# SakodaShintaro/f2-nerf

Measured on AMD Instinct MI355X. Metric: rendered rays/sec (fwd+bwd) at 800x800, higher is better.
Workload: dtype f32; 1 GPU; ngp_fox-like synthetic views 800x800, 128 samples/ray, L=16 F=2 T=2^19, 65536-ray chunks, TRAIN render + loss + backward (optimizer excluded); pixel_order=rows, regime=dense

## Files before the change

### f2-nerf_amd/csrc/host/ragged_ops.cpp

```cpp
#include "ragged_ops.hpp"

#include "kernel_timer.hpp"

using torch::Tensor;
using torch::autograd::AutogradContext;
using torch::autograd::variable_list;

namespace
{

class FlexSumFn : public torch::autograd::Function<FlexSumFn>
{
public:
  static variable_list forward(AutogradContext * ctx, Tensor val, Tensor idx)
  {
    val = f2n::dev_f32(val, "FlexOps::Sum val");
    idx = f2n::dev_i32(idx, "FlexOps::Sum idx_start_end");
    TORCH_CHECK(val.dim() == 1 || val.dim() == 2, "FlexOps::Sum expects [n] or [n, c]");
    const int n_rays = (int)idx.size(0);
    void * s = f2n::current_stream(val);
    Tensor sum;
    if (val.dim() == 1) {
      sum = torch::empty({n_rays}, val.options());
      f2n::check(
        f2n_seg_sum_fwd(f2n::fptr(val), f2n::iptr(idx), sum.data_ptr<float>(), n_rays, s),
        "f2n_seg_sum_fwd");
    } else {
      const int vec = (int)val.size(1);
      sum = torch::empty({n_rays, vec}, val.options());
      f2n::check(
        f2n_seg_sum_vec_fwd(f2n::fptr(val), f2n::iptr(idx), sum.data_ptr<float>(), n_rays, vec, s),
        "f2n_seg_sum_vec_fwd");
    }
    ctx->save_for_backward({idx});
    ctx->saved_data["n_all"] = (int64_t)val.size(0);
    ctx->saved_data["vec"] = (int64_t)(val.dim() == 1 ? 0 : val.size(1));
    return {sum};
  }

  static variable_list backward(AutogradContext * ctx, variable_list grad_output)
  {
    Tensor dsum = f2n::dev_f32(grad_output[0], "FlexOps::Sum grad");
    Tensor idx = ctx->get_saved_variables()[0];
    const int64_t n_all = ctx->saved_data["n_all"].toInt();
    const int vec = (int)ctx->saved_data["vec"].toInt();
    const int n_rays = (int)idx.size(0);
    void * s = f2n::current_stream(dsum);
    Tensor dval;
    if (vec == 0) {
      dval = torch::zeros({n_all}, dsum.options());
      f2n::check(
        f2n_seg_sum_bwd(f2n::fptr(dsum), f2n::iptr(idx), dval.data_ptr<float>(), n_rays, s),
        "f2n_seg_sum_bwd");
    } else {
      dval = torch::zeros({n_all, vec}, dsum.options());
      f2n::check(
        f2n_seg_sum_vec_bwd(f2n::fptr(dsum), f2n::iptr(idx), dval.data_ptr<float>(), n_rays, vec, s),
        "f2n_seg_sum_vec_bwd");
    }
    return {dval, Tensor()};
  }
};

class FlexAccumulateSumFn : public torch::autograd::Function<FlexAccumulateSumFn>
{
public:
  static variable_list forward(AutogradContext * ctx, Tensor val, Tensor idx, bool include_this)
  {
    val = f2n::dev_f32(val, "FlexOps::AccumulateSum val");
    idx = f2n::dev_i32(idx, "FlexOps::AccumulateSum idx_start_end");
    TORCH_CHECK(val.dim() == 1, "FlexOps::AccumulateSum expects [n]");
    Tensor sum = torch::zeros_like(val);
    f2n::check(
      f2n_seg_scan_fwd(
        f2n::fptr(val), f2n::iptr(idx), sum.data_ptr<float>(), (int)idx.size(0), include_this,
        f2n::current_stream(val)),
      "f2n_seg_scan_fwd");
    ctx->save_for_backward({idx});
    ctx->saved_data["include_this"] = include_this;
    return {sum};
  }

  static variable_list backward(AutogradContext * ctx, variable_list grad_output)
  {
    Tensor dsum = f2n::dev_f32(grad_output[0], "FlexOps::AccumulateSum grad");
    Tensor idx = ctx->get_saved_variables()[0];
    const bool include_this = ctx->saved_data["include_this"].toBool();
    Tensor dval = torch::zeros_like(dsum);
    f2n::check(
      f2n_seg_scan_bwd(
        f2n::fptr(dsum), f2n::iptr(idx), dval.data_ptr<float>(), (int)idx.size(0), include_this,
        f2n::current_stream(dsum)),
      "f2n_seg_scan_bwd");
    return {dval, Tensor(), Tensor()};
  }
};

class WeightVarFn : public torch::autograd::Function<WeightVarFn>
{
public:
  static variable_list forward(AutogradContext * ctx, Tensor weights, Tensor idx)
  {
    weights = f2n::dev_f32(weights, "CustomOps::WeightVar weights");
    idx = f2n::dev_i32(idx, "CustomOps::WeightVar idx_start_end");
    const int n_rays = (int)idx.size(0);
    Tensor out = torch::empty({n_rays}, weights.options());
    f2n::check(
      f2n_weight_var_fwd(
        f2n::fptr(weights), f2n::iptr(idx), out.data_ptr<float>(), n_rays,
        f2n::current_stream(weights)),
      "f2n_weight_var_fwd");
    ctx->save_for_backward({weights, idx});
    return {out};
  }

  static variable_list backward(AutogradContext * ctx, variable_list grad_output)
  {
    Tensor dvar = f2n::dev_f32(grad_output[0], "CustomOps::WeightVar grad");
    auto saved = ctx->get_saved_variables();
    Tensor & weights = saved[0];
    Tensor & idx = saved[1];
    Tensor dw = torch::zeros_like(weights);
    f2n::check(
      f2n_weight_var_bwd(
        f2n::fptr(weights), f2n::iptr(idx), f2n::fptr(dvar), dw.data_ptr<float>(),
        (int)idx.size(0), f2n::current_stream(dvar)),
      "f2n_weight_var_bwd");
    return {dw, Tensor()};
  }
};

class ScatterAddFn : public torch::autograd::Function<ScatterAddFn>
{
public:
  static variable_list forward(AutogradContext * ctx, Tensor emb, Tensor idx, Tensor to_add)
  {
    emb = f2n::dev_f32(emb, "CustomOps::ScatterAdd emb");
    idx = f2n::dev_i32(idx, "CustomOps::ScatterAdd idx");
    to_add = f2n::dev_f32(to_add, "CustomOps::ScatterAdd to_add");
    const int64_t n_all = idx.size(0);
    const int C = (int)emb.size(1);
    TORCH_CHECK(to_add.size(0) == n_all && to_add.size(1) == C, "ScatterAdd shape mismatch");
    Tensor sum = torch::empty_like(to_add);
    f2n::check(
      f2n_scatter_add_fwd(
        f2n::fptr(emb), f2n::iptr(idx), f2n::fptr(to_add), sum.data_ptr<float>(), n_all, C,
        f2n::current_stream(to_add)),
      "f2n_scatter_add_fwd");
    ctx->save_for_backward({idx});
    ctx->saved_data["n_emb"] = (int64_t)emb.size(0);
    return {sum};
  }

  static variable_list backward(AutogradContext * ctx, variable_list grad_output)
  {
    Tensor dsum = f2n::dev_f32(grad_output[0], "CustomOps::ScatterAdd grad");
    Tensor idx = ctx->get_saved_variables()[0];
    const int n_emb = (int)ctx->saved_data["n_emb"].toInt();
    const int C = (int)dsum.size(1);
    Tensor demb = torch::empty({n_emb, C}, dsum.options());
    f2n::check(
      f2n_scatter_add_bwd(
        f2n::iptr(idx), f2n::fptr(dsum), demb.data_ptr<float>(), idx.size(0), n_emb, C,
        f2n::current_stream(dsum)),
      "f2n_scatter_add_bwd");
    return {demb, Tensor(), dsum};
  }
};

class CompositeFn : public torch::autograd::Function<CompositeFn>
{
public:
  static variable_list forward(
    AutogradContext * ctx, Tensor field_out, Tensor rgb, Tensor dt, Tensor t, Tensor idx, Tensor bg,
    bool tiled)
  {
    field_out = f2n::dev_f32(field_out, "composite field_out");
    rgb = f2n::dev_f32(rgb, "composite rgb");
    dt = f2n::dev_f32(dt, "composite dt");
    t = f2n::dev_f32(t, "composite t");
    idx = f2n::dev_i32(idx, "composite idx_start_end");
    bg = f2n::dev_f32(bg, "composite bg_color");
    TORCH_CHECK(field_out.dim() == 2 && rgb.dim() == 2 && rgb.size(1) == 3, "composite shapes");
    const int64_t n = field_out.size(0);
    const int n_rays = (int)idx.size(0);
    auto opt = field_out.options();
    Tensor colors = torch::empty({n_rays, 3}, opt), depths = torch::empty({n_rays}, opt);
    Tensor weights = tiled ? torch::empty({n}, opt) : torch::zeros({n}, opt);
    Tensor last_trans = torch::empty({n_rays}, opt);
    ctx->saved_data["tiled"] = tiled;
    f2n::check(
      f2n_composite_fwd(
        f2n::fptr(field_out), field_out.size(1), f2n::fptr(rgb), f2n::fptr(dt), f2n::fptr(t),
        f2n::iptr(idx), f2n::fptr(bg), colors.data_ptr<float>(), depths.data_ptr<float>(),
        weights.data_ptr<float>(), last_trans.data_ptr<float>(), n_rays, 3.f, 1e-2f,
        f2n::current_stream(field_out)),
      "f2n_composite_fwd");
    ctx->save_for_backward({field_out, rgb, dt, t, idx, bg, weights, last_trans});
    return {colors, depths, weights};
  }

  static variable_list backward(AutogradContext * ctx, variable_list grad_output)
  {
    auto sv = ctx->get_saved_variables();
    Tensor &field_out = sv[0], &rgb = sv[1], &dt = sv[2], &t = sv[3], &idx = sv[4], &bg = sv[5],
           &weights = sv[6], &last_trans = sv[7];
    const int n_rays = (int)idx.size(0);
    const int64_t n = field_out.size(0);
    auto opt = field_out.options();
    Tensor d_colors = grad_output[0].defined() ? f2n::dev_f32(grad_output[0], "d_colors")
                                               : torch::zeros({n_rays, 3}, opt);
    Tensor d_depths = grad_output[1].defined() ? f2n::dev_f32(grad_output[1], "d_depths")
                                               : torch::zeros({n_rays}, opt);
    Tensor d_weights =
      grad_output[2].defined() ? f2n::dev_f32(grad_output[2], "d_weights") : Tensor();
    const bool tiled = ctx->saved_data["tiled"].toBool();
    Tensor d_logit = tiled ? torch::empty({n}, opt) : torch::zeros({n}, opt);
    Tensor d_rgb = tiled ? torch::empty({n, 3}, opt) : torch::zeros({n, 3}, opt);
    f2n::check(
      f2n_composite_bwd(
        f2n::fptr(field_out), field_out.size(1), f2n::fptr(rgb), f2n::fptr(dt), f2n::fptr(t),
        f2n::iptr(idx), f2n::fptr(bg), f2n::fptr(weights), f2n::fptr(last_trans),
        f2n::fptr(d_colors), f2n::fptr(d_depths), f2n::fptr(d_weights), d_logit.data_ptr<float>(),
        d_rgb.data_ptr<float>(), n_rays, 3.f, 1e-2f, f2n::current_stream(field_out)),
      "f2n_composite_bwd");
    if (field_out.size(1) == 1)
      return {d_logit.unsqueeze(1), d_rgb, Tensor(), Tensor(), Tensor(), Tensor(), Tensor()};
    Tensor d_field = torch::zeros_like(field_out);
    d_field.select(1, 0).copy_(d_logit);
    return {d_field, d_rgb, Tensor(), Tensor(), Tensor(), Tensor(), Tensor()};
  }
};

Tensor as_channel_major(const Tensor & t)
{
  if (t.dim() == 2 && t.stride(0) == 1 && t.stride(1) == t.size(0)) return t.t();
  return t.t().contiguous();
}

class ShadeFn : public torch::autograd::Function<ShadeFn>
{
public:
  static variable_list forward(
    AutogradContext * ctx, Tensor enc, Tensor dirs, Tensor sample_img, Tensor w_h, Tensor b_h,
    Tensor w1, Tensor b1, Tensor w2, Tensor b2, Tensor app_emb)
  {
    TORCH_CHECK(enc.is_cuda() && enc.scalar_type() == torch::kFloat32 && enc.dim() == 2, "enc");
    const int64_t n = enc.size(0);
    const int C = (int)enc.size(1);
    Tensor enc_cm = as_channel_major(enc);
    dirs = f2n::dev_f32(dirs.detach(), "shade dirs");
    const bool use_emb = sample_img.defined() && app_emb.defined() && sample_img.numel() > 0 &&
                         app_emb.numel() > 0;
    if (use_emb) sample_img = f2n::dev_i32(sample_img, "shade sample_img");
    w_h = f2n::dev_f32(w_h, "w_h");
    b_h = f2n::dev_f32(b_h, "b_h");
    w1 = f2n::dev_f32(w1, "w1");
    b1 = f2n::dev_f32(b1, "b1");
    w2 = f2n::dev_f32(w2, "w2");
    b2 = f2n::dev_f32(b2, "b2");
    Tensor emb = use_emb ? f2n::dev_f32(app_emb, "app_emb") : Tensor();
    TORCH_CHECK(
      w_h.size(0) == 16 && w_h.size(1) == C && w1.size(0) == 64 && w1.size(1) == 32 &&
        w2.size(0) == 3 && w2.size(1) == 64,
      "shade: layer shapes must be 16xC, 64x32, 3x64");
    Tensor logit = torch::empty({n}, enc.options()), rgb = torch::empty({n, 3}, enc.options());
    {
    f2n::ScopedKernelTimer timer("shade_fwd", f2n::current_stream(enc_cm), (double)n);
    f2n::check(
      f2n_shade_fwd(
        enc_cm.data_ptr<float>(), C, dirs.data_ptr<float>(), use_emb ? f2n::iptr(sample_img) : nullptr,
        f2n::fptr(w_h), f2n::fptr(b_h), f2n::fptr(w1), f2n::fptr(b1), f2n::fptr(w2), f2n::fptr(b2),
        f2n::fptr(emb), logit.data_ptr<float>(), rgb.data_ptr<float>(),
        nullptr,
        n, f2n::current_stream(enc_cm)),
      "f2n_shade_fwd");
    }
    ctx->save_for_backward(
      {enc_cm, dirs, use_emb ? sample_img : Tensor(), w_h, b_h, w1, b1, w2, b2, emb});
    return {logit, rgb};
  }

  static variable_list backward(AutogradContext * ctx, variable_list grad_output)
  {
    auto sv = ctx->get_saved_variables();
    Tensor &enc_cm = sv[0], &dirs = sv[1], &sample_img = sv[2], &w_h = sv[3], &b_h = sv[4],
           &w1 = sv[5], &b1 = sv[6], &w2 = sv[7], &b2 = sv[8], &emb = sv[9];
    const int C = (int)enc_cm.size(0);
    const int64_t n = enc_cm.size(1);
    auto opt = enc_cm.options();
    Tensor d_logit = grad_output[0].defined() ? f2n::dev_f32(grad_output[0], "d_logit")
                                              : torch::zeros({n}, opt);
    Tensor d_rgb = grad_output[1].defined() ? f2n::dev_f32(grad_output[1], "d_rgb")
                                            : torch::zeros({n, 3}, opt);
    Tensor d_enc_cm = torch::empty({(int64_t)C, n}, opt);
    const bool use_emb = emb.defined() && sample_img.defined();
    auto pad4 = [](int64_t v) { return (v + 3) / 4 * 4; };
    const int64_t sizes[7] = {w_h.numel(), b_h.numel(), w1.numel(), b1.numel(),
                              w2.numel(), b2.numel(), use_emb ? emb.numel() : 0};
    int64_t total = 0;
    for (int64_t v : sizes) total += pad4(v);
    Tensor gbuf = torch::zeros({total}, opt);
    int64_t off = 0;
    auto take = [&](const Tensor & like, int64_t numel) {
      Tensor v = gbuf.narrow(0, off, numel).view(like.sizes());
      off += pad4(numel);
      return v;
    };
    Tensor g_w_h = take(w_h, sizes[0]), g_b_h = take(b_h, sizes[1]), g_w1 = take(w1, sizes[2]),
           g_b1 = take(b1, sizes[3]), g_w2 = take(w2, sizes[4]), g_b2 = take(b2, sizes[5]);
    Tensor g_emb = use_emb ? take(emb, sizes[6]) : Tensor();
    {
    f2n::ScopedKernelTimer timer("shade_bwd", f2n::current_stream(enc_cm), (double)n);
    f2n::check(
      f2n_shade_bwd(
        enc_cm.data_ptr<float>(), C, dirs.data_ptr<float>(), use_emb ? f2n::iptr(sample_img) : nullptr,
        f2n::fptr(w_h), f2n::fptr(b_h), f2n::fptr(w1), f2n::fptr(b1), f2n::fptr(w2), f2n::fptr(b2),
        f2n::fptr(emb), f2n::fptr(d_logit), f2n::fptr(d_rgb), d_enc_cm.data_ptr<float>(),
        g_w_h.data_ptr<float>(), g_b_h.data_ptr<float>(), g_w1.data_ptr<float>(),
        g_b1.data_ptr<float>(), g_w2.data_ptr<float>(), g_b2.data_ptr<float>(),
        use_emb ? g_emb.data_ptr<float>() : nullptr, nullptr, n,
        f2n::current_stream(enc_cm)),
      "f2n_shade_bwd");
    }
    return {d_enc_cm.t(), Tensor(), Tensor(), g_w_h, g_b_h, g_w1, g_b1, g_w2, g_b2, g_emb};
  }
};


class TrainLossFn : public torch::autograd::Function<TrainLossFn>
{
public:
  static variable_list forward(
    AutogradContext * ctx, Tensor colors, Tensor gt, Tensor var, double var_weight)
  {
    colors = f2n::dev_f32(colors, "train_loss colors");
    gt = f2n::dev_f32(gt, "train_loss gt_colors");
    var = f2n::dev_f32(var, "train_loss var");
    const int64_t n_rays = colors.size(0);
    TORCH_CHECK(
      colors.dim() == 2 && colors.size(1) == 3 && gt.sizes() == colors.sizes() &&
        var.numel() == n_rays && n_rays > 0 && n_rays <= INT32_MAX,
      "train_loss: colors/gt [n_rays,3], var [n_rays]");
    Tensor d_colors = torch::empty_like(colors), d_var = torch::empty({n_rays}, colors.options());
    Tensor partial = torch::empty({f2n_loss_workspace_floats((int)n_rays)}, colors.options());
    Tensor out = torch::empty({4}, colors.options());
    f2n::check(
      f2n_loss_fwd(
        colors.data_ptr<float>(), gt.data_ptr<float>(), var.data_ptr<float>(), (int)n_rays,
        (float)var_weight, d_colors.data_ptr<float>(), d_var.data_ptr<float>(),
        partial.data_ptr<float>(), out.data_ptr<float>(), f2n::current_stream(colors)),
      "f2n_loss_fwd");
    ctx->save_for_backward({d_colors, d_var});
    ctx->saved_data["var_shape"] = var.sizes().vec();
    return {out};
  }

  static variable_list backward(AutogradContext * ctx, variable_list grad_output)
  {
    auto sv = ctx->get_saved_variables();
    Tensor g = grad_output[0].select(0, 0);
    Tensor d_var = (sv[1] * g).view(ctx->saved_data["var_shape"].toIntVector());
    return {sv[0] * g, Tensor(), d_var, Tensor()};
  }
};

}

namespace torch::autograd
{

variable_list TruncExp::forward(AutogradContext * ctx, Tensor input)
{
  ctx->save_for_backward({input});
  return {torch::exp(input)};
}

variable_list TruncExp::backward(AutogradContext * ctx, variable_list grad_output)
{
  Tensor x = ctx->get_saved_variables()[0];
  return {grad_output[0] * torch::exp(x.clamp(-100.f, 5.f))};
}

}

Tensor FlexOps::Sum(Tensor val, Tensor idx_start_end)
{
  return FlexSumFn::apply(val.contiguous(), idx_start_end.contiguous())[0];
}

Tensor FlexOps::AccumulateSum(Tensor val, Tensor idx_start_end, bool include_this)
{
  return FlexAccumulateSumFn::apply(val.contiguous(), idx_start_end.contiguous(), include_this)[0];
}

Tensor CustomOps::WeightVar(Tensor weights, Tensor idx_start_end)
{
  return WeightVarFn::apply(weights.contiguous(), idx_start_end.contiguous())[0];
}

Tensor CustomOps::ScatterAdd(Tensor emb, Tensor idx, Tensor to_add)
{
  return ScatterAddFn::apply(emb, idx, to_add)[0];
}

Tensor CustomOps::ScatterIdx(int n_all_pts, Tensor idx_start_end, Tensor emb_idx)
{
  idx_start_end = f2n::dev_i32(idx_start_end, "CustomOps::ScatterIdx idx_start_end");
  emb_idx = f2n::dev_i32(emb_idx, "CustomOps::ScatterIdx emb_idx");
  Tensor ret = torch::empty({n_all_pts}, idx_start_end.options());
  f2n::check(
    f2n_scatter_idx(
      f2n::iptr(idx_start_end), f2n::iptr(emb_idx), ret.data_ptr<int32_t>(),
      (int)idx_start_end.size(0), f2n::current_stream(idx_start_end)),
    "f2n_scatter_idx");
  return ret;
}

f2n::ShadeOut f2n::shade(
  const Tensor & enc, const Tensor & dirs, const Tensor & sample_img, const Tensor & w_h,
  const Tensor & b_h, const Tensor & w1, const Tensor & b1, const Tensor & w2, const Tensor & b2,
  const Tensor & app_emb)
{
  const Tensor no_img = torch::empty({0}, f2n::int_on(enc.device()));
  const Tensor no_emb = torch::empty({0, 16}, enc.options());
  const bool use_emb = sample_img.defined() && app_emb.defined();
  auto out = ShadeFn::apply(
    enc, dirs, use_emb ? sample_img : no_img, w_h, b_h, w1, b1, w2, b2, use_emb ? app_emb : no_emb);
  return {out[0], out[1]};
}

f2n::CompositeOut f2n::composite(
  const Tensor & field_out, const Tensor & rgb, const Tensor & dt, const Tensor & t,
  const Tensor & idx_start_end, const Tensor & bg_color, bool bounds_tile_samples)
{
  auto out = CompositeFn::apply(field_out, rgb, dt, t, idx_start_end, bg_color, bounds_tile_samples);
  return {out[0], out[1], out[2]};
}

Tensor f2n::train_loss(
  const Tensor & colors, const Tensor & gt_colors, const Tensor & var, float var_loss_weight)
{
  return TrainLossFn::apply(colors, gt_colors, var, (double)var_loss_weight)[0];
}
```

### f2-nerf_amd/csrc/host/ragged_ops.hpp

```cpp
#pragma once

#include "common.hpp"

namespace torch::autograd
{

class TruncExp : public Function<TruncExp>
{
public:
  static variable_list forward(AutogradContext * ctx, Tensor input);
  static variable_list backward(AutogradContext * ctx, variable_list grad_output);
};

}

namespace FlexOps
{
torch::Tensor Sum(torch::Tensor val, torch::Tensor idx_start_end);
torch::Tensor AccumulateSum(torch::Tensor val, torch::Tensor idx_start_end, bool include_this);
}

namespace CustomOps
{
torch::Tensor WeightVar(torch::Tensor weights, torch::Tensor idx_start_end);
torch::Tensor ScatterAdd(torch::Tensor emb, torch::Tensor idx, torch::Tensor to_add);
torch::Tensor ScatterIdx(int n_all_pts, torch::Tensor idx_start_end, torch::Tensor emb_idx);
}

namespace f2n
{

struct CompositeOut
{
  Tensor colors;
  Tensor depths;
  Tensor weights;
};

CompositeOut composite(
  const Tensor & field_out, const Tensor & rgb, const Tensor & dt, const Tensor & t,
  const Tensor & idx_start_end, const Tensor & bg_color, bool bounds_tile_samples = false);


struct ShadeOut
{
  Tensor logit;
  Tensor rgb;
};

ShadeOut shade(
  const Tensor & enc, const Tensor & dirs, const Tensor & sample_img, const Tensor & w_h,
  const Tensor & b_h, const Tensor & w1, const Tensor & b1, const Tensor & w2, const Tensor & b2,
  const Tensor & app_emb);

Tensor train_loss(
  const Tensor & colors, const Tensor & gt_colors, const Tensor & var, float var_loss_weight);

inline bool shade_supported(int64_t C) { return C == 8 || C == 16 || C == 32 || C == 64; }

}
```

### f2-nerf_amd/csrc/host/renderer.cpp

```cpp
#include "renderer.hpp"

#include "kernel_timer.hpp"

#include "ragged_ops.hpp"
#include "rays.hpp"

#include <c10/hip/HIPGuard.h>
#include <hip/hip_runtime_api.h>

using Tensor = torch::Tensor;

f2n::HostCount::~HostCount()
{
  if (event_) hipEventDestroy((hipEvent_t)event_);
  if (pinned_) hipHostFree(pinned_);
}

void f2n::HostCount::request(const torch::Tensor & device_int32, void * stream)
{
  TORCH_CHECK(
    device_int32.is_cuda() && device_int32.scalar_type() == torch::kInt32 && device_int32.numel() == 1,
    "HostCount: one int32 on the device");
  const int device = (int)device_int32.device().index();
  c10::hip::HIPGuard on_device(device);
  if (pending_) {
    hipEventSynchronize((hipEvent_t)event_);
    pending_ = false;
  }
  if (!pinned_)
    TORCH_CHECK(hipHostMalloc((void **)&pinned_, sizeof(int32_t), hipHostMallocDefault) == hipSuccess,
                "HostCount: pinned allocation failed");
  if (!event_ || device_ != device) {
    if (event_) hipEventDestroy((hipEvent_t)event_);
    hipEvent_t ev;
    TORCH_CHECK(hipEventCreateWithFlags(&ev, hipEventDisableTiming) == hipSuccess,
                "HostCount: event creation failed");
    event_ = ev;
    device_ = device;
  }
  TORCH_CHECK(
    hipMemcpyAsync(pinned_, device_int32.data_ptr<int32_t>(), sizeof(int32_t), hipMemcpyDeviceToHost,
                   (hipStream_t)stream) == hipSuccess &&
      hipEventRecord((hipEvent_t)event_, (hipStream_t)stream) == hipSuccess,
    "HostCount: copy failed");
  pending_ = true;
}

int64_t f2n::HostCount::wait()
{
  TORCH_CHECK(pending_, "HostCount: wait() without request()");
  TORCH_CHECK(hipEventSynchronize((hipEvent_t)event_) == hipSuccess, "HostCount: wait failed");
  pending_ = false;
  return (int64_t)*pinned_;
}


namespace
{

std::pair<Tensor, Tensor> bounds_from_counts(const Tensor & counts, void * stream)
{
  const int n = (int)counts.size(0);
  Tensor bounds = torch::empty({n, 2}, counts.options()), total = torch::empty({1}, counts.options());
  f2n::check(
    f2n_bounds_from_counts(
      counts.data_ptr<int32_t>(), bounds.data_ptr<int32_t>(), total.data_ptr<int32_t>(), n, stream),
    "f2n_bounds_from_counts");
  return {bounds, total};
}

class RayUnpermuteFn : public torch::autograd::Function<RayUnpermuteFn>
{
public:
  static torch::autograd::variable_list forward(
    torch::autograd::AutogradContext * ctx, Tensor colors, Tensor depths, Tensor weights,
    Tensor perm, Tensor inv, Tensor bounds_sorted, Tensor bounds_caller, int64_t S, bool rows)
  {
    colors = f2n::dev_f32(colors, "colors");
    depths = f2n::dev_f32(depths, "depths");
    weights = f2n::dev_f32(weights, "weights");
    const int n = (int)perm.size(0);
    void * s = f2n::current_stream(colors);
    Tensor c = torch::empty_like(colors), d = torch::empty_like(depths), w = torch::empty_like(weights);
    gather(colors, depths, weights, c, d, w, inv, bounds_sorted, bounds_caller, n, S, rows, s);
    ctx->save_for_backward({perm, bounds_sorted, bounds_caller});
    ctx->saved_data["S"] = S;
    ctx->saved_data["rows"] = rows;
    return {c, d, w};
  }

  static torch::autograd::variable_list backward(
    torch::autograd::AutogradContext * ctx, torch::autograd::variable_list g)
  {
    auto saved = ctx->get_saved_variables();
    const Tensor & perm = saved[0];
    const int n = (int)perm.size(0);
    const int64_t S = ctx->saved_data["S"].toInt();
    const bool rows = ctx->saved_data["rows"].toBool();
    Tensor gc = g[0].defined() ? f2n::dev_f32(g[0], "grad colors") : Tensor();
    Tensor gd = g[1].defined() ? f2n::dev_f32(g[1], "grad depths") : Tensor();
    Tensor gw = g[2].defined() ? f2n::dev_f32(g[2], "grad weights") : Tensor();
    Tensor dc = gc.defined() ? torch::empty_like(gc) : Tensor();
    Tensor dd = gd.defined() ? torch::empty_like(gd) : Tensor();
    Tensor dw = gw.defined() ? torch::empty_like(gw) : Tensor();
    void * s = f2n::current_stream(perm);
    gather(gc, gd, gw, dc, dd, dw, perm, saved[2], saved[1], n, S, rows, s);
    return {dc, dd, dw, Tensor(), Tensor(), Tensor(), Tensor(), Tensor(), Tensor()};
  }

private:
  static void gather(
    const Tensor & c, const Tensor & d, const Tensor & w, Tensor & c_out, Tensor & d_out,
    Tensor & w_out, const Tensor & map, const Tensor & src_b, const Tensor & dst_b, int n, int64_t S,
    bool rows, void * s)
  {
    const int32_t * m = map.data_ptr<int32_t>();
    if (c.defined())
      f2n::check(f2n_gather_rows(f2n::fptr(c), c_out.data_ptr<float>(), m, n, 3, s), "f2n_gather_rows");
    if (d.defined())
      f2n::check(f2n_gather_rows(f2n::fptr(d), d_out.data_ptr<float>(), m, n, 1, s), "f2n_gather_rows");
    if (!w.defined()) return;
    if (rows)
      f2n::check(
        f2n_gather_rows(f2n::fptr(w), w_out.data_ptr<float>(), m, n, (int)S, s), "f2n_gather_rows");
    else
      f2n::check(
        f2n_gather_segments(
          f2n::fptr(w), f2n::iptr(src_b), w_out.data_ptr<float>(), f2n::iptr(dst_b), m, n, s),
        "f2n_gather_segments");
  }
};

class RayGradFn : public torch::autograd::Function<RayGradFn>
{
public:
  static torch::autograd::variable_list forward(
    torch::autograd::AutogradContext * ctx, Tensor enc, Tensor rays_o, Tensor rays_d, Tensor pts,
    Tensor t, Tensor bounds, torch::IValue hash3d_info)
  {
    Hash3DAnchored * field = hash3d_info.toCustomClass<Hash3DAnchoredInfo>()->hash3d_;
    ctx->saved_data["hash3d_info"] = hash3d_info;
    ctx->saved_data["n_rays"] = rays_o.size(0);
    ctx->save_for_backward(
      {f2n::dev_f32(pts.detach(), "kept pts"), f2n::dev_f32(t.detach(), "kept t"),
       f2n::dev_i32(bounds, "kept bounds"), f2n::dev_f32(rays_d.detach(), "rays_d"),
       field->table_f16()});
    return {enc};
  }

  static torch::autograd::variable_list backward(
    torch::autograd::AutogradContext * ctx, torch::autograd::variable_list grad)
  {
    const Tensor & g_enc = grad[0];
    const bool want_o = ctx->needs_input_grad(1), want_d = ctx->needs_input_grad(2);
    Tensor d_o, d_d;
    if (want_o || want_d) {
      auto sv = ctx->get_saved_variables();
      const Tensor &pts = sv[0], &t = sv[1], &bounds = sv[2], &rays_d = sv[3], &table16 = sv[4];
      const int64_t n_rays = ctx->saved_data["n_rays"].toInt();
      d_o = torch::empty({n_rays, 3}, rays_d.options());
      d_d = torch::empty({n_rays, 3}, rays_d.options());
      if (!g_enc.defined()) {
        d_o.zero_();
        d_d.zero_();
      } else {
        Hash3DAnchored * field =
          ctx->saved_data["hash3d_info"].toCustomClass<Hash3DAnchoredInfo>()->hash3d_;
        const int64_t n = pts.size(0);
        const int L = (int)field->options_.n_levels, F = (int)field->options_.n_channels;
        const auto [g, ld_point, ld_chan] = f2n::encoding_grad_strides(g_enc, n, (int64_t)L * F);
        void * stream = f2n::current_stream(pts);
        f2n::ScopedKernelTimer timer("hash_rays_grad", stream, (double)n);
        f2n::check(
          f2n_hash_rays_grad(
            pts.data_ptr<float>(), t.data_ptr<float>(), bounds.data_ptr<int32_t>(),
            rays_d.data_ptr<float>(), reinterpret_cast<const uint16_t *>(table16.data_ptr()),
            field->prim_pool_.data_ptr<int32_t>(), field->bias_pool_.data_ptr<float>(),
            field->level_mul_.data_ptr<float>(), g.data_ptr<float>(), ld_point, ld_chan,
            d_o.data_ptr<float>(), d_d.data_ptr<float>(), (int)n_rays, L, F,
            (uint32_t)field->local_size_, field->level_stride_, 128.f ,
            stream),
          "f2n_hash_rays_grad");
      }
    }
    return {g_enc, want_o ? d_o : Tensor(), want_d ? d_d : Tensor(), Tensor(), Tensor(), Tensor(),
            Tensor()};
  }
};

}

Tensor f2n::ray_order(const Tensor & rays_d_in)
{
  const Tensor rays_d = f2n::dev_f32(rays_d_in.detach(), "rays_d");
  TORCH_CHECK(rays_d.dim() == 2 && rays_d.size(1) == 3, "rays_d must be [n, 3]");
  const int n = (int)rays_d.size(0);
  Tensor keys = torch::empty({n}, f2n::int_on(rays_d.device()));
  f2n::check(
    f2n_ray_keys(rays_d.data_ptr<float>(), keys.data_ptr<int32_t>(), n, f2n::current_stream(rays_d)),
    "f2n_ray_keys");
  return std::get<1>(keys.sort(true, 0, false));
}

Renderer::Renderer(int n_images, const RendererOptions & opt) : options_(opt)
{
  pts_sampler_ = std::make_shared<PtsSampler>(opt.sampler);

  scene_field_ = std::make_shared<Hash3DAnchored>(opt.field);
  register_module("scene_field", scene_field_);

  shader_ = std::make_shared<SHShader>(opt.field.device);
  register_module("shader", shader_);

  app_emb_ = torch::randn({n_images, 16}, f2n::float_on(opt.field.device)) * .1f;
  app_emb_.requires_grad_(true);
  register_parameter("app_emb", app_emb_);
}

RenderResult Renderer::render(
  const Tensor & rays_o, const Tensor & rays_d, const Tensor & emb_idx, RunningMode mode)
{
  return render(rays_o, rays_d, emb_idx, mode, Tensor(), Tensor());
}

RenderResult Renderer::render(
  const Tensor & rays_o, const Tensor & rays_d, const Tensor & emb_idx, RunningMode mode,
  const Tensor & noise_in, const Tensor & bg_in)
{
  const int64_t n_rays = rays_o.size(0);
  const auto fopt = f2n::float_on(rays_o.device());
  Tensor noise = noise_in.defined() ? noise_in
                                    : pts_sampler_->draw_noise(n_rays, mode, rays_o.device());
  Tensor bg_color = bg_in.defined() ? bg_in
                    : (mode == RunningMode::TRAIN) ? torch::rand({n_rays, 3}, fopt)
                                                   : torch::ones({n_rays, 3}, fopt) * .5f;
  if (n_rays <= 0) {
    record_kept(0);
    return {bg_color, torch::zeros({n_rays}, fopt), torch::full({n_rays}, 512.f, fopt), Tensor()};
  }
  const Route route = choose_route(rays_o, rays_d, bg_color);
  RenderResult res = route.first_pass == Route::OpByOp
                       ? render_op_by_op(rays_o, rays_d, emb_idx, mode, noise, bg_color, route)
                       : render_fused(rays_o, rays_d, emb_idx, mode, noise, bg_color, route);
  if (options_.check_finite) CHECK(std::isfinite(res.colors.mean().item<float>()));
  return res;
}

Renderer::Route Renderer::choose_route(
  const Tensor & rays_o, const Tensor & rays_d, const Tensor & bg_color) const
{
  Route route;
  const auto & field = scene_field_->options_;
  route.fused_net = options_.fused_shade && f2n::shade_supported(field.n_levels * field.n_channels) &&
                    field.mlp_out_dim == 16;
  const bool rays_need_grad =
    torch::GradMode::is_enabled() && (rays_o.requires_grad() || rays_d.requires_grad());
  if (rays_need_grad) route.grad_rays = Rays{rays_o, rays_d};
  if (!options_.fused || (rays_need_grad && !(options_.fused_ray_grad && route.fused_net)))
    route.first_pass = Route::OpByOp;
  else if (occupancy_)
    route.first_pass = Route::March;
  else if (route.fused_net && (options_.dense_first_pass == 1 ||
                               (options_.dense_first_pass < 0 && last_kept_fraction_ > 0.4f)))
    route.first_pass = Route::Dense;
  else
    route.first_pass = Route::March;
  route.bucketed = route.first_pass == Route::Dense &&
                   rays_o.size(0) >= options_.ray_order_min_rays &&
                   f2n_get_option(F2N_OPT_RAY_ORDER) == 0 && !rays_need_grad &&
                   !(torch::GradMode::is_enabled() && bg_color.requires_grad());
  return route;
}

void Renderer::record_kept(int64_t n_kept, int64_t n_all)
{
  last_n_samples_ = n_kept;
  if (n_all >= 0) last_kept_fraction_ = n_all > 0 ? (float)n_kept / (float)n_all : 0.f;
}


RenderResult Renderer::render_op_by_op(
  const Tensor & rays_o, const Tensor & rays_d, const Tensor & emb_idx, RunningMode mode,
  const Tensor & noise, const Tensor & bg_color, const Route & route)
{
  const int64_t n_rays = rays_o.size(0);
  const int64_t S = pts_sampler_->options_.max_samples;
  SampleResultFlex all = route.grad_rays.origins.defined()
                           ? pts_sampler_->get_samples_aten(rays_o, rays_d, noise)
                           : pts_sampler_->get_samples(rays_o, rays_d, noise);

  auto density_act = [](const Tensor & x) {
    return torch::autograd::TruncExp::apply(x - 3.f)[0];
  };

  SampleResultFlex kept;
  {
    Tensor scene_feat = scene_field_->query(all.pts);
    Tensor density = density_act(scene_feat.index({Slc(), Slc(0, 1)}));
    Tensor sec = density.index({Slc(), 0}) * all.dt;
    Tensor occupied;
    if (occupancy_) {
      occupied = occupancy_->occupied(all.pts);
      sec = sec * occupied.to(sec.scalar_type());
    }
    Tensor acc = FlexOps::AccumulateSum(sec, all.pts_idx_bounds, false);
    Tensor mask = torch::exp(-acc) > options_.early_stop_trans;
    if (occupancy_) mask = mask.logical_and(occupied);
    Tensor mask_idx = torch::where(mask)[0];
    kept.pts = all.pts.index({mask_idx}).contiguous();
    kept.dirs = all.dirs.index({mask_idx}).contiguous();
    kept.dt = all.dt.index({mask_idx}).contiguous();
    kept.t = all.t.index({mask_idx}).contiguous();
    Tensor num = mask.reshape({n_rays, S}).sum(1);
    Tensor cum = torch::cumsum(num, 0);
    kept.pts_idx_bounds = torch::stack({cum - num, cum}, 1).to(torch::kInt32).contiguous();
  }
  record_kept(kept.pts.size(0));

  Tensor scene_feat = scene_field_->query(kept.pts);
  Tensor density = density_act(scene_feat.index({Slc(), Slc(0, 1)}));
  Tensor sampled_colors = shade_aten(scene_feat, kept, emb_idx, mode);
  Tensor sampled_t = (kept.t + 1e-2f).contiguous();
  Tensor sec = density.index({Slc(), 0}) * kept.dt;
  Tensor alphas = 1.f - torch::exp(-sec);
  Tensor idx = kept.pts_idx_bounds;
  Tensor trans = torch::exp(-FlexOps::AccumulateSum(sec, idx, false));
  Tensor weights = trans * alphas;
  Tensor last_trans = torch::exp(-FlexOps::Sum(sec, idx));
  Tensor colors = FlexOps::Sum(weights.unsqueeze(-1) * sampled_colors, idx) +
                  last_trans.unsqueeze(-1) * bg_color;
  Tensor depths = FlexOps::Sum(weights * sampled_t, idx) / (1.f - last_trans + 1e-4f);
  return {colors, depths, weights, idx};
}


RenderResult Renderer::render_fused(
  const Tensor & rays_o_raw, const Tensor & rays_d_raw, const Tensor & emb_idx, RunningMode mode,
  const Tensor & noise_raw, const Tensor & bg_color, const Route & route)
{
  Tensor rays_o = f2n::dev_f32(rays_o_raw.detach(), "rays_o");
  Tensor rays_d = f2n::dev_f32(rays_d_raw.detach(), "rays_d");
  Tensor noise = noise_raw.defined() ? f2n::dev_f32(noise_raw, "noise") : Tensor();
  const int n_rays = (int)rays_o.size(0);
  const int S = pts_sampler_->options_.max_samples;
  TORCH_CHECK(!noise.defined() || noise.numel() == (int64_t)n_rays * S, "noise shape");
  if (route.first_pass == Route::Dense)
    return route.bucketed
             ? render_dense_bucketed(rays_o, rays_d, emb_idx, mode, noise, bg_color, route)
             : render_dense(rays_o, rays_d, emb_idx, mode, noise, bg_color, route);

  void * stream = f2n::current_stream(rays_o);
  Hash3DAnchored & field = *scene_field_;
  SampleResultFlex kept;
  {
    torch::NoGradGuard no_grad;
    Tensor table16 = field.table_f16();
    auto head = field.density_head();
    Tensor counts = torch::empty({n_rays}, f2n::int_on(rays_o.device()));
    Tensor len;
    if (occupancy_) {
      TORCH_CHECK(
        occupancy_->words().device() == rays_o.device(), "the occupancy grid lives on another device");
      len = torch::empty_like(counts);
      f2n::ScopedKernelTimer timer("density_march_occ", stream, (double)n_rays);
      f2n::check(
        f2n_density_march_occ(
          rays_o.data_ptr<float>(), rays_d.data_ptr<float>(), f2n::fptr(noise),
          reinterpret_cast<const uint16_t *>(table16.data_ptr()),
          field.prim_pool_.data_ptr<int32_t>(), field.bias_pool_.data_ptr<float>(),
          field.level_mul_.data_ptr<float>(), head.first.data_ptr<float>(),
          head.second.data_ptr<float>(), occupancy_->words_ptr(), (int)occupancy_->resolution(),
          counts.data_ptr<int32_t>(), len.data_ptr<int32_t>(), n_rays, S,
          pts_sampler_->options_.step, (int)field.options_.n_levels, (int)field.options_.n_channels,
          (uint32_t)field.local_size_, field.level_stride_, options_.early_stop_trans, 3.f, stream),
        "f2n_density_march_occ");
    } else {
      f2n::ScopedKernelTimer timer("density_march", stream, (double)n_rays);
      f2n::check(
      f2n_density_march(
        rays_o.data_ptr<float>(), rays_d.data_ptr<float>(), f2n::fptr(noise),
        reinterpret_cast<const uint16_t *>(table16.data_ptr()), field.prim_pool_.data_ptr<int32_t>(),
        field.bias_pool_.data_ptr<float>(), field.level_mul_.data_ptr<float>(),
        head.first.data_ptr<float>(), head.second.data_ptr<float>(), counts.data_ptr<int32_t>(),
        n_rays, S, pts_sampler_->options_.step, (int)field.options_.n_levels,
        (int)field.options_.n_channels, (uint32_t)field.local_size_, field.level_stride_,
        options_.early_stop_trans, 3.f, stream),
      "f2n_density_march");
    }
    auto [bounds, total] = bounds_from_counts(counts, stream);
    const int64_t n_kept = total.item<int>();
    record_kept(n_kept, (int64_t)n_rays * S);
    kept = compact_samples(rays_o, rays_d, noise, bounds, n_kept, len);
  }
  return shade_and_composite(kept, emb_idx, mode, bg_color, route);
}

RenderResult Renderer::render_dense_bucketed(
  const Tensor & rays_o, const Tensor & rays_d, const Tensor & emb_idx_in, RunningMode mode,
  const Tensor & noise, const Tensor & bg_in, const Route & route)
{
  const int n_rays = (int)rays_o.size(0);
  const int64_t S = pts_sampler_->options_.max_samples;
  const auto iopt = f2n::int_on(rays_o.device());
  void * stream = f2n::current_stream(rays_o);
  const Tensor emb_idx = (mode == RunningMode::TRAIN && emb_idx_in.defined())
                           ? f2n::dev_i32(emb_idx_in, "emb_idx") : Tensor();
  const Tensor bg = f2n::dev_f32(bg_in.detach(), "bg_color");
  TORCH_CHECK(bg.numel() == (int64_t)n_rays * 3, "bg_color shape");
  TORCH_CHECK(!emb_idx.defined() || emb_idx.numel() == n_rays, "emb_idx shape");

  const Tensor order = f2n::ray_order(rays_d);
  Tensor perm = torch::empty({n_rays}, iopt), inv = torch::empty({n_rays}, iopt);
  Tensor o_p = torch::empty_like(rays_o), d_p = torch::empty_like(rays_d), bg_p = torch::empty_like(bg);
  Tensor emb_p = emb_idx.defined() ? torch::empty_like(emb_idx) : Tensor();
  Tensor noise_p = noise.defined() ? torch::empty_like(noise) : Tensor();
  f2n::check(
    f2n_ray_permute(
      order.data_ptr<int64_t>(), n_rays, (int)S, rays_o.data_ptr<float>(), rays_d.data_ptr<float>(),
      f2n::iptr(emb_idx), bg.data_ptr<float>(), f2n::fptr(noise), perm.data_ptr<int32_t>(),
      o_p.data_ptr<float>(), d_p.data_ptr<float>(),
      emb_idx.defined() ? emb_p.data_ptr<int32_t>() : nullptr, bg_p.data_ptr<float>(),
      f2n::fptr_mut(noise_p), inv.data_ptr<int32_t>(), stream),
    "f2n_ray_permute");
  RenderResult r = render_dense(o_p, d_p, emb_p, mode, noise_p, bg_p, route);

  const bool rows = r.weights.size(0) == (int64_t)n_rays * S;
  Tensor bounds = r.idx_start_end;
  if (!rows) {
    Tensor counts = torch::empty({n_rays}, iopt);
    f2n::check(
      f2n_counts_through(
        r.idx_start_end.data_ptr<int32_t>(), inv.data_ptr<int32_t>(), counts.data_ptr<int32_t>(),
        n_rays, stream),
      "f2n_counts_through");
    bounds = bounds_from_counts(counts, stream).first;
  }
  auto out = RayUnpermuteFn::apply(
    r.colors, r.depths, r.weights, perm, inv, r.idx_start_end, bounds, S, rows);
  return {out[0], out[1], out[2], bounds};
}

RenderResult Renderer::render_dense(
  const Tensor & rays_o, const Tensor & rays_d, const Tensor & emb_idx, RunningMode mode,
  const Tensor & noise, const Tensor & bg_color, const Route & route)
{
  const int n_rays = (int)rays_o.size(0);
  const int S = pts_sampler_->options_.max_samples;
  void * stream = f2n::current_stream(rays_o);
  Hash3DAnchored & field = *scene_field_;
  SampleResultFlex all = pts_sampler_->get_samples(rays_o, rays_d, noise);
  const int64_t n_all = all.pts.size(0);
  Tensor contracted_all, enc_all_cm;
  {
    torch::NoGradGuard no_grad;
    enc_all_cm = field.encode(all.pts, S, &contracted_all).t();
    TORCH_CHECK(enc_all_cm.is_contiguous(), "encode() must return channel-major storage");
  }

  if (options_.deferred_check) {
    Tensor total = scan_survivors(all, enc_all_cm, n_rays).second;
    if (!deferred_bad_.defined()) deferred_bad_ = torch::zeros({1}, total.options());
    deferred_bad_.add_(total.ne(n_all).to(torch::kInt32));
    record_kept(n_all, n_all);
    return shade_and_composite(all, emb_idx, mode, bg_color, route, enc_all_cm, contracted_all);
  }

  const bool may_guess = options_.speculate_dense && last_kept_fraction_ >= 1.f && n_all > 0;
  const bool large = n_all >= options_.margin_min_samples;
  if (may_guess && large) {
    if (auto guess = shade_all_unless_near_threshold(
          all, emb_idx, mode, bg_color, route, enc_all_cm, contracted_all)) {
      record_kept(n_all, n_all);
      return *guess;
    }
  }

  auto [bounds, total] = scan_survivors(all, enc_all_cm, n_rays);
  survivors_.request(total, stream);
  RenderResult guess;
  const bool guessed = may_guess && !large;
  if (guessed)
    guess = shade_and_composite(all, emb_idx, mode, bg_color, route, enc_all_cm, contracted_all);
  const int64_t n_kept = survivors_.wait();
  record_kept(n_kept, n_all);
  if (guessed && n_kept == n_all) return guess;
  guess = RenderResult();
  if (n_kept == n_all) {
    all.pts_idx_bounds = bounds;
    return shade_and_composite(all, emb_idx, mode, bg_color, route, enc_all_cm, contracted_all);
  }
  SampleResultFlex kept = compact_samples(rays_o, rays_d, noise, bounds, n_kept);
  const int64_t C = enc_all_cm.size(0);
  Tensor enc_kept_cm = torch::empty({C, n_kept}, rays_o.options());
  f2n::check(
    f2n_compact_rows_cm(
      enc_all_cm.data_ptr<float>(), n_all, enc_kept_cm.data_ptr<float>(), n_kept, (int)C,
      bounds.data_ptr<int32_t>(), n_rays, S, stream),
    "f2n_compact_rows_cm");
  return shade_and_composite(kept, emb_idx, mode, bg_color, route, enc_kept_cm);
}

bool Renderer::deferred_check_ok()
{
  if (!deferred_bad_.defined()) return true;
  const bool ok = deferred_bad_.item<int32_t>() == 0;
  deferred_bad_.zero_();
  return ok;
}


std::pair<Tensor, Tensor> Renderer::scan_survivors(
  const SampleResultFlex & all, const Tensor & enc_all_cm, int n_rays)
{
  torch::NoGradGuard no_grad;
  void * stream = f2n::current_stream(enc_all_cm);
  auto head = scene_field_->density_head();
  Tensor counts = torch::empty({n_rays}, f2n::int_on(enc_all_cm.device()));
  {
    f2n::ScopedKernelTimer timer("density_scan", stream, (double)n_rays);
    f2n::check(
      f2n_density_scan(
        enc_all_cm.data_ptr<float>(), (int)enc_all_cm.size(0), all.dt.data_ptr<float>(),
        head.first.data_ptr<float>(), head.second.data_ptr<float>(), counts.data_ptr<int32_t>(),
        n_rays, pts_sampler_->options_.max_samples, options_.early_stop_trans, 3.f, stream),
      "f2n_density_scan");
  }
  return bounds_from_counts(counts, stream);
}

SampleResultFlex Renderer::compact_samples(
  const Tensor & rays_o, const Tensor & rays_d, const Tensor & noise, const Tensor & bounds,
  int64_t n_kept, const Tensor & len)
{
  const auto fopt = rays_o.options();
  SampleResultFlex kept{
    torch::empty({n_kept, 3}, fopt), torch::empty({n_kept, 3}, fopt), torch::empty({n_kept}, fopt),
    torch::empty({n_kept}, fopt), bounds};
  if (len.defined()) {
    f2n::check(
      f2n_sample_compact_occ(
        rays_o.data_ptr<float>(), rays_d.data_ptr<float>(), f2n::fptr(noise),
        bounds.data_ptr<int32_t>(), len.data_ptr<int32_t>(), occupancy_->words_ptr(),
        (int)occupancy_->resolution(), kept.pts.data_ptr<float>(), kept.dirs.data_ptr<float>(),
        kept.dt.data_ptr<float>(), kept.t.data_ptr<float>(), (int)rays_o.size(0),
        pts_sampler_->options_.max_samples, pts_sampler_->options_.step,
        f2n::current_stream(rays_o)),
      "f2n_sample_compact_occ");
    return kept;
  }
  f2n::check(
    f2n_sample_compact(
      rays_o.data_ptr<float>(), rays_d.data_ptr<float>(), f2n::fptr(noise),
      bounds.data_ptr<int32_t>(), kept.pts.data_ptr<float>(), kept.dirs.data_ptr<float>(),
      kept.dt.data_ptr<float>(), kept.t.data_ptr<float>(), (int)rays_o.size(0),
      pts_sampler_->options_.max_samples, pts_sampler_->options_.step,
      f2n::current_stream(rays_o)),
    "f2n_sample_compact");
  return kept;
}

std::optional<RenderResult> Renderer::shade_all_unless_near_threshold(
  const SampleResultFlex & all, const Tensor & emb_idx, RunningMode mode, const Tensor & bg_color,
  const Route & route, const Tensor & enc_cm, const Tensor & contracted)
{
  void * stream = f2n::current_stream(all.pts);
  Tensor near_threshold = torch::zeros({1}, f2n::int_on(all.pts.device()));
  Shaded shaded = shade(all, emb_idx, mode, route, enc_cm, contracted);
  const int S = pts_sampler_->options_.max_samples;
  const float limit = -std::log(options_.early_stop_trans) - 0.5f;
  f2n::check(
    f2n_density_margin(
      shaded.field_out.data_ptr<float>(), all.dt.data_ptr<float>(),
      near_threshold.data_ptr<int32_t>(), (int)(all.pts.size(0) / S), S, 3.f, limit, stream),
    "f2n_density_margin");
  survivors_.request(near_threshold, stream);
  RenderResult guess = composite(all, shaded, bg_color, route);
  if (survivors_.wait() != 0) return std::nullopt;
  return guess;
}

RenderResult Renderer::shade_and_composite(
  const SampleResultFlex & kept, const Tensor & emb_idx, RunningMode mode, const Tensor & bg_color,
  const Route & route, const Tensor & enc_cm, const Tensor & contracted)
{
  return composite(kept, shade(kept, emb_idx, mode, route, enc_cm, contracted), bg_color, route);
}

Renderer::Shaded Renderer::shade(
  const SampleResultFlex & kept, const Tensor & emb_idx, RunningMode mode, const Route & route,
  const Tensor & enc_cm, const Tensor & contracted)
{
  if (!route.fused_net) {
    Tensor scene_feat = scene_field_->query(kept.pts);
    return {scene_feat, shade_aten(scene_feat, kept, emb_idx, mode)};
  }
  const int64_t n_kept = kept.pts.size(0);
  Tensor enc = enc_cm.defined() ? scene_field_->encode_cached(kept.pts, enc_cm, contracted)
                                : scene_field_->encode(kept.pts);
  if (route.grad_rays.origins.defined()) {
    auto info = torch::make_intrusive<Hash3DAnchoredInfo>();
    info->hash3d_ = scene_field_.get();
    enc = RayGradFn::apply(
      enc, route.grad_rays.origins, route.grad_rays.dirs, kept.pts, kept.t, kept.pts_idx_bounds,
      torch::IValue(info))[0];
  }
  Tensor sample_img;
  if (mode == RunningMode::TRAIN)
    sample_img = CustomOps::ScatterIdx((int)n_kept, kept.pts_idx_bounds, emb_idx);
  auto mlp = shader_->mlp_params();
  f2n::ShadeOut sh = f2n::shade(
    enc, kept.dirs, sample_img, scene_field_->mlp_->weight, scene_field_->mlp_->bias, mlp[0],
    mlp[1], mlp[2], mlp[3], mode == RunningMode::TRAIN ? app_emb_ : Tensor());
  return {sh.logit.unsqueeze(1), sh.rgb};
}

Tensor Renderer::shade_aten(
  const Tensor & scene_feat, const SampleResultFlex & kept, const Tensor & emb_idx, RunningMode mode)
{
  const int64_t n_kept = kept.pts.size(0);
  Tensor shading_feat = torch::cat(
    {torch::ones({n_kept, 1}, scene_feat.options()),
     scene_feat.index({Slc(), Slc(1, torch::indexing::None)})},
    1);
  if (mode == RunningMode::TRAIN) {
    Tensor all_emb_idx = CustomOps::ScatterIdx((int)n_kept, kept.pts_idx_bounds, emb_idx);
    shading_feat = CustomOps::ScatterAdd(app_emb_, all_emb_idx, shading_feat);
  }
  return shader_->query(shading_feat, kept.dirs);
}

RenderResult Renderer::composite(
  const SampleResultFlex & kept, const Shaded & shaded, const Tensor & bg_color, const Route & route)
{
  f2n::CompositeOut out = f2n::composite(
    shaded.field_out, shaded.rgb, kept.dt, kept.t, kept.pts_idx_bounds, bg_color, route.fused_net);
  return {out.colors, out.depths, out.weights, kept.pts_idx_bounds};
}


std::tuple<Tensor, Tensor> Renderer::render_all_rays(
  const Tensor & rays_o, const Tensor & rays_d, const int batch_size)
{
  const int64_t n_rays = rays_d.size(0);
  std::vector<Tensor> colors, depths;
  for (int64_t lo = 0; lo < n_rays; lo += batch_size) {
    const int64_t hi = std::min<int64_t>(lo + batch_size, n_rays);
    RenderResult r = render(
      rays_o.index({Slc(lo, hi)}).contiguous(), rays_d.index({Slc(lo, hi)}).contiguous(), Tensor(),
      RunningMode::VALIDATE);
    colors.push_back(r.colors);
    depths.push_back(r.depths.reshape({-1, 1}));
  }
  return {torch::cat(colors, 0), torch::cat(depths, 0)};
}

std::tuple<Tensor, Tensor> Renderer::render_image(
  const Tensor & pose, const Tensor & intrinsic, const int h, const int w, const int batch_size)
{
  Rays rays = get_view_rays(pose, intrinsic, h, w);
  const int B = options_.pixel_tiles;
  Tensor order;
  if (B > 1 && h % B == 0 && w % B == 0) {
    order = torch::arange((int64_t)h * w, torch::TensorOptions().dtype(torch::kInt64).device(pose.device()))
              .view({h / B, B, w / B, B})
              .permute({0, 2, 1, 3})
              .reshape({-1});
    rays.origins = rays.origins.index_select(0, order);
    rays.dirs = rays.dirs.index_select(0, order);
  }
  auto [colors, depths] = render_all_rays(rays.origins, rays.dirs, batch_size);
  if (order.defined()) {
    colors = torch::empty_like(colors).index_copy_(0, order, colors);
    depths = torch::empty_like(depths).index_copy_(0, order, depths);
  }
  colors = colors.reshape({h, w, 3}).clip(0.f, 1.f);
  depths = depths.reshape({h, w, 1}).repeat({1, 1, 3});
  return {colors, depths};
}

std::vector<torch::optim::OptimizerParamGroup> Renderer::optim_param_groups(float lr)
{
  std::vector<torch::optim::OptimizerParamGroup> groups;
  for (auto & g : scene_field_->optim_param_groups(lr)) groups.emplace_back(g);
  for (auto & g : shader_->optim_param_groups(lr)) groups.emplace_back(g);
  auto opt = std::make_unique<torch::optim::AdamOptions>(lr);
  opt->betas(std::make_tuple(0.9, 0.99)).eps(1e-15).weight_decay(1e-6);
  groups.emplace_back(std::vector<Tensor>{app_emb_}, std::move(opt));
  return groups;
}


f2n::TrainStepResult f2n::train_step(
  Renderer & renderer, const Tensor & rays_o, const Tensor & rays_d, const Tensor & emb_idx,
  const Tensor & gt_colors, float var_loss_weight, const Tensor & noise, const Tensor & bg_color,
  bool run_backward)
{
  RenderResult res =
    renderer.render(rays_o, rays_d, emb_idx, RunningMode::TRAIN, noise, bg_color);
  Tensor var = CustomOps::WeightVar(res.weights, res.idx_start_end);
  if (var_loss_weight == 0.f) var = var.detach();
  Tensor stats = f2n::train_loss(res.colors, gt_colors, var, var_loss_weight);
  Tensor loss = stats[0];
  TrainStepResult out;
  out.loss = loss.detach();
  out.sq_err_sum = stats[3].detach();
  out.n_values = res.colors.numel();
  out.n_samples = renderer.last_n_samples_;
  if (run_backward && loss.requires_grad()) loss.backward();
  return out;
}
```

### f2-nerf_amd/csrc/kernels/shade.hip

```cpp
#include "sh_basis.hiph"
#include "shade_mfma.hiph"

#include <cstdlib>
#include <cstring>

namespace
{

constexpr int kOut1 = 16;
constexpr int kIn2 = 32;
constexpr int kHid = 64;
constexpr float kEps = 1e-3f;

struct ShadeParams
{
  const float * __restrict__ w_h;
  const float * __restrict__ b_h;
  const float * __restrict__ w1;
  const float * __restrict__ b1;
  const float * __restrict__ w2;
  const float * __restrict__ b2;
  const float * __restrict__ emb;
};

template <int C>
__device__ __forceinline__ void shade_forward(
  const float (&e)[C], float dx, float dy, float dz, const float * __restrict__ emb_row,
  const ShadeParams & P, float (&h)[kOut1], float (&X)[kIn2], float (&pre)[kHid], float (&o)[3])
{
#pragma unroll
  for (int i = 0; i < kOut1; i++) {
    float acc = P.b_h[i];
#pragma unroll
    for (int c = 0; c < C; c++) acc = fmaf(e[c], P.w_h[i * C + c], acc);
    h[i] = acc;
  }
  X[0] = 1.f;
#pragma unroll
  for (int i = 1; i < kOut1; i++) X[i] = h[i];
  if (emb_row) {
#pragma unroll
    for (int i = 0; i < kOut1; i++) X[i] += emb_row[i];
  }
  sh_basis<4>(dx, dy, dz, &X[kOut1]);
#pragma unroll
  for (int j = 0; j < kHid; j++) {
    float acc = P.b1[j];
#pragma unroll
    for (int i = 0; i < kIn2; i++) acc = fmaf(X[i], P.w1[j * kIn2 + i], acc);
    pre[j] = acc;
  }
#pragma unroll
  for (int c = 0; c < 3; c++) {
    float acc = P.b2[c];
#pragma unroll
    for (int j = 0; j < kHid; j++) acc = fmaf(fmaxf(pre[j], 0.f), P.w2[c * kHid + j], acc);
    o[c] = acc;
  }
}

template <int C>
__global__ __launch_bounds__(F2N_BLOCK) void shade_fwd_kernel(
  const float * __restrict__ enc, const float * __restrict__ dirs,
  const int32_t * __restrict__ sample_img, const float * __restrict__ p_w_h,
  const float * __restrict__ p_b_h, const float * __restrict__ p_w1,
  const float * __restrict__ p_b1, const float * __restrict__ p_w2,
  const float * __restrict__ p_b2, const float * __restrict__ p_emb, float * __restrict__ logit,
  float * __restrict__ rgb, float * __restrict__ pre_out, int64_t n)
{
  const int64_t p = (int64_t)blockIdx.x * F2N_BLOCK + threadIdx.x;
  if (p >= n) return;
  const ShadeParams P{p_w_h, p_b_h, p_w1, p_b1, p_w2, p_b2, p_emb};
  float e[C];
#pragma unroll
  for (int c = 0; c < C; c++) e[c] = enc[(int64_t)c * n + p];
  const float * emb_row = (P.emb && sample_img) ? P.emb + (int64_t)sample_img[p] * kOut1 : nullptr;
  float h[kOut1], X[kIn2], pre[kHid], o[3];
  shade_forward<C>(e, dirs[3 * p], dirs[3 * p + 1], dirs[3 * p + 2], emb_row, P, h, X, pre, o);
  logit[p] = h[0];
#pragma unroll
  for (int c = 0; c < 3; c++)
    rgb[3 * p + c] = (1.f + 2.f * kEps) / (1.f + expf(-o[c])) - kEps;
  if (pre_out) {
#pragma unroll
    for (int j = 0; j < kHid; j++) pre_out[(int64_t)j * n + p] = pre[j];
  }
}


constexpr int kTP = 65;
constexpr int kDoOff = kHid * kTP;
constexpr int kHP = kOut1 + 4;

template <int C>
struct BwdShape
{
  static constexpr int kERowP = C + 4;
  static constexpr int kHOff = 64 * kERowP;
  static constexpr int kTile =
    (kHOff + 64 * kHP > kDoOff + 64 * 3) ? kHOff + 64 * kHP : kDoOff + 64 * 3;
  static constexpr int kWeights = kOut1 * (C + 4) + kHid * (kIn2 + 4) + kHid * 4 + 4;
  static constexpr int kWaves = ((kWeights + 8 * kTile) * 4 <= 160 * 1024) ? 8 : 4;
};

__device__ __forceinline__ void wave_lds_sync()
{
  __builtin_amdgcn_fence(__ATOMIC_RELEASE, "wavefront");
  __builtin_amdgcn_wave_barrier();
  __builtin_amdgcn_fence(__ATOMIC_ACQUIRE, "wavefront");
}

template <int C>
__global__ __launch_bounds__(BwdShape<C>::kWaves * 64) void shade_bwd_kernel(
  const float * __restrict__ enc, const float * __restrict__ dirs,
  const int32_t * __restrict__ sample_img, const float * __restrict__ p_w_h,
  const float * __restrict__ p_b_h, const float * __restrict__ p_w1,
  const float * __restrict__ p_b1, const float * __restrict__ p_w2,
  const float * __restrict__ p_b2, const float * __restrict__ p_emb,
  const float * __restrict__ d_logit, const float * __restrict__ d_rgb, float * __restrict__ d_enc,
  float * __restrict__ g_w_h, float * __restrict__ g_b_h, float * __restrict__ g_w1,
  float * __restrict__ g_b1, float * __restrict__ g_w2, float * __restrict__ g_b2,
  float * __restrict__ g_emb, const float * __restrict__ pre_in, int64_t n)
{
  static_assert(C % 4 == 0 && C <= kHid, "C must be a multiple of 4 and at most 64");
  constexpr int kBwdWaves = BwdShape<C>::kWaves;
  constexpr int kWavelds = BwdShape<C>::kTile;
  constexpr int kWhP = C + 4, kW1P = kIn2 + 4;
  constexpr int kOffWh = 0, kOffW1 = kOffWh + kOut1 * kWhP, kOffW2T = kOffW1 + kHid * kW1P,
                kOffB2 = kOffW2T + kHid * 4, kWTotal = kOffB2 + 4;
  __shared__ __attribute__((aligned(16))) float lds_all[kWTotal + kBwdWaves * kWavelds];
  float * lds_w = lds_all;
  float * lds = lds_all + kWTotal;
  for (int i = threadIdx.x; i < kOut1 * C; i += kBwdWaves * 64)
    lds_w[kOffWh + (i / C) * kWhP + (i % C)] = p_w_h[i];
  for (int i = threadIdx.x; i < kHid * kIn2; i += kBwdWaves * 64)
    lds_w[kOffW1 + (i / kIn2) * kW1P + (i % kIn2)] = p_w1[i];
  for (int i = threadIdx.x; i < 3 * kHid; i += kBwdWaves * 64)
    lds_w[kOffW2T + (i % kHid) * 4 + (i / kHid)] = p_w2[i];
  if (threadIdx.x < kOut1) lds_w[kOffWh + threadIdx.x * kWhP + C] = p_b_h[threadIdx.x];
  if (threadIdx.x < kHid) {
    lds_w[kOffW1 + threadIdx.x * kW1P + kIn2] = p_b1[threadIdx.x];
    lds_w[kOffW2T + threadIdx.x * 4 + 3] = 0.f;
  }
  if (threadIdx.x < 4) lds_w[kOffB2 + threadIdx.x] = (threadIdx.x < 3) ? p_b2[threadIdx.x] : 0.f;
  __syncthreads();

  const int lane = lane_id();
  const int wave = (int)(threadIdx.x >> 6);
  int vzero;
  asm volatile("v_mov_b32 %0, 0" : "=v"(vzero));
  float * tileP = lds + wave * kWavelds;
  const bool has_emb = (p_emb != nullptr) && (sample_img != nullptr);

  float acc_w1[kIn2];
  float acc_b1 = 0.f;
  float acc_w2[3];
  constexpr int CQ = C / 4;
  float acc_wh[CQ];
  float acc_bh[kOut1];
  float acc_b2[3];
#pragma unroll
  for (int i = 0; i < kIn2; i++) acc_w1[i] = 0.f;
#pragma unroll
  for (int c = 0; c < 3; c++) acc_w2[c] = acc_b2[c] = 0.f;
#pragma unroll
  for (int k = 0; k < CQ; k++) acc_wh[k] = 0.f;
#pragma unroll
  for (int i = 0; i < kOut1; i++) acc_bh[i] = 0.f;

  const int64_t n_strides = (n + 63) / 64;
  const int64_t wave_global = (int64_t)blockIdx.x * kBwdWaves + wave;
  const int64_t wave_count = (int64_t)gridDim.x * kBwdWaves;
  for (int64_t st = wave_global; st < n_strides; st += wave_count) {
    const int64_t p = st * 64 + lane;
    const bool valid = p < n;
    const int64_t pc = valid ? p : n - 1;

    float e[C];
#pragma unroll
    for (int c = 0; c < C; c++) e[c] = enc[(int64_t)c * n + pc];
    const int img = has_emb ? sample_img[pc] : 0;
    float X[kIn2];
    {
#pragma unroll 2
      for (int i = 0; i < kOut1; i++) {
        const float * row = lds_w + kOffWh + (i + vzero) * kWhP;
        float acc = row[C];
#pragma unroll
        for (int c = 0; c < C; c += 4) {
          const float4 w = *reinterpret_cast<const float4 *>(row + c);
          acc = fmaf(e[c], w.x, acc);
          acc = fmaf(e[c + 1], w.y, acc);
          acc = fmaf(e[c + 2], w.z, acc);
          acc = fmaf(e[c + 3], w.w, acc);
        }
        tileP[i * 64 + lane] = acc;
      }
      X[0] = 1.f;
#pragma unroll
      for (int i = 1; i < kOut1; i++) X[i] = tileP[i * 64 + lane];
      if (has_emb) {
        const float * emb_row = p_emb + (int64_t)img * kOut1;
#pragma unroll
        for (int i = 0; i < kOut1; i++) X[i] += emb_row[i];
      }
      sh_basis<4>(dirs[3 * pc], dirs[3 * pc + 1], dirs[3 * pc + 2], &X[kOut1]);
    }
    float o[3];
    {
      const float4 b2 = *reinterpret_cast<const float4 *>(lds_w + kOffB2);
      o[0] = b2.x;
      o[1] = b2.y;
      o[2] = b2.z;
      if (pre_in) {
#pragma unroll 8
        for (int j = 0; j < kHid; j++) {
          const float acc = pre_in[(int64_t)j * n + pc];
          tileP[j * kTP + lane] = acc;
          const float hj = fmaxf(acc, 0.f);
          const float4 w2 = *reinterpret_cast<const float4 *>(lds_w + kOffW2T + (j + vzero) * 4);
          o[0] = fmaf(hj, w2.x, o[0]);
          o[1] = fmaf(hj, w2.y, o[1]);
          o[2] = fmaf(hj, w2.z, o[2]);
        }
      } else {
#pragma unroll 2
        for (int j = 0; j < kHid; j++) {
          const float * row = lds_w + kOffW1 + (j + vzero) * kW1P;
          float acc = row[kIn2];
#pragma unroll
          for (int i = 0; i < kIn2; i += 4) {
            const float4 w = *reinterpret_cast<const float4 *>(row + i);
            acc = fmaf(X[i], w.x, acc);
            acc = fmaf(X[i + 1], w.y, acc);
            acc = fmaf(X[i + 2], w.z, acc);
            acc = fmaf(X[i + 3], w.w, acc);
          }
          tileP[j * kTP + lane] = acc;
          const float hj = fmaxf(acc, 0.f);
          const float4 w2 = *reinterpret_cast<const float4 *>(lds_w + kOffW2T + (j + vzero) * 4);
          o[0] = fmaf(hj, w2.x, o[0]);
          o[1] = fmaf(hj, w2.y, o[1]);
          o[2] = fmaf(hj, w2.z, o[2]);
        }
      }
    }

    float d_o[3];
#pragma unroll
    for (int c = 0; c < 3; c++) {
      const float sg = 1.f / (1.f + expf(-o[c]));
      const float g = valid ? d_rgb[3 * pc + c] : 0.f;
      d_o[c] = g * (1.f + 2.f * kEps) * sg * (1.f - sg);
      acc_b2[c] += d_o[c];
    }

    tileP[kDoOff + lane * 3 + 0] = d_o[0];
    tileP[kDoOff + lane * 3 + 1] = d_o[1];
    tileP[kDoOff + lane * 3 + 2] = d_o[2];
    wave_lds_sync();
#pragma unroll 4
    for (int s = 0; s < 64; s++) {
      const float a = fmaxf(tileP[lane * kTP + s], 0.f);
      const float * g = tileP + kDoOff + (s + vzero) * 3;
      acc_w2[0] = fmaf(g[0], a, acc_w2[0]);
      acc_w2[1] = fmaf(g[1], a, acc_w2[1]);
      acc_w2[2] = fmaf(g[2], a, acc_w2[2]);
    }
    wave_lds_sync();

    float dX[kOut1];
#pragma unroll
    for (int i = 0; i < kOut1; i++) dX[i] = 0.f;
#pragma unroll 2
    for (int j = 0; j < kHid; j++) {
      const float pre = tileP[j * kTP + lane];
      const float4 w2 = *reinterpret_cast<const float4 *>(lds_w + kOffW2T + (j + vzero) * 4);
      float dh = d_o[0] * w2.x;
      dh = fmaf(d_o[1], w2.y, dh);
      dh = fmaf(d_o[2], w2.z, dh);
      dh = (pre > 0.f) ? dh : 0.f;
      tileP[j * kTP + lane] = dh;
      const float * row = lds_w + kOffW1 + (j + vzero) * kW1P;
#pragma unroll
      for (int i = 0; i < kOut1; i += 4) {
        const float4 w = *reinterpret_cast<const float4 *>(row + i);
        dX[i] = fmaf(dh, w.x, dX[i]);
        dX[i + 1] = fmaf(dh, w.y, dX[i + 1]);
        dX[i + 2] = fmaf(dh, w.z, dX[i + 2]);
        dX[i + 3] = fmaf(dh, w.w, dX[i + 3]);
      }
    }
    float d_h[kOut1];
    d_h[0] = valid ? d_logit[pc] : 0.f;
#pragma unroll
    for (int i = 1; i < kOut1; i++) d_h[i] = dX[i];
#pragma unroll
    for (int i = 0; i < kOut1; i++) acc_bh[i] += d_h[i];

    wave_lds_sync();
#pragma unroll 2
    for (int s = 0; s < 64; s++) {
      const float a = tileP[lane * kTP + s];
      acc_b1 += a;
#pragma unroll
      for (int i = 0; i < kIn2; i++) {
        const float xs =
          __int_as_float(__builtin_amdgcn_readlane(__float_as_int(X[i]), s));
        acc_w1[i] = fmaf(a, xs, acc_w1[i]);
      }
    }
    wave_lds_sync();

    {
      float d_e[C];
#pragma unroll
      for (int c = 0; c < C; c++) d_e[c] = 0.f;
#pragma unroll
      for (int i = 0; i < kOut1; i++) tileP[i * 64 + lane] = d_h[i];
#pragma unroll 2
      for (int i = 0; i < kOut1; i++) {
        const float a = tileP[i * 64 + lane];
        const float * row = lds_w + kOffWh + (i + vzero) * kWhP;
#pragma unroll
        for (int c = 0; c < C; c += 4) {
          const float4 w = *reinterpret_cast<const float4 *>(row + c);
          d_e[c] = fmaf(a, w.x, d_e[c]);
          d_e[c + 1] = fmaf(a, w.y, d_e[c + 1]);
          d_e[c + 2] = fmaf(a, w.z, d_e[c + 2]);
          d_e[c + 3] = fmaf(a, w.w, d_e[c + 3]);
        }
      }
      if (valid) {
#pragma unroll
        for (int c = 0; c < C; c++) d_enc[(int64_t)c * n + p] = d_e[c];
      }
    }

    {
      constexpr int kEP = BwdShape<C>::kERowP;
      float * rowsH = tileP + BwdShape<C>::kHOff;
      wave_lds_sync();
#pragma unroll
      for (int c = 0; c < C; c += 4)
        *reinterpret_cast<float4 *>(tileP + lane * kEP + c) =
          make_float4(e[c], e[c + 1], e[c + 2], e[c + 3]);
      *reinterpret_cast<float4 *>(rowsH + lane * kHP) =
        make_float4(valid ? dX[0] : 0.f, d_h[1], d_h[2], d_h[3]);
#pragma unroll
      for (int i = 4; i < kOut1; i += 4)
        *reinterpret_cast<float4 *>(rowsH + lane * kHP + i) =
          make_float4(d_h[i], d_h[i + 1], d_h[i + 2], d_h[i + 3]);
      rowsH[lane * kHP + kOut1] = d_h[0];
      wave_lds_sync();
      const int wi = lane & 15, wq = lane >> 4;
      const int col = (wi == 0) ? kOut1 : wi;
#pragma unroll 4
      for (int s = 0; s < 64; s++) {
        const float a = rowsH[s * kHP + col];
#pragma unroll
        for (int k = 0; k < CQ; k += 4) {
          const float4 x = *reinterpret_cast<const float4 *>(tileP + s * kEP + wq * CQ + k);
          acc_wh[k] = fmaf(a, x.x, acc_wh[k]);
          if (k + 1 < CQ) acc_wh[k + 1] = fmaf(a, x.y, acc_wh[k + 1]);
          if (k + 2 < CQ) acc_wh[k + 2] = fmaf(a, x.z, acc_wh[k + 2]);
          if (k + 3 < CQ) acc_wh[k + 3] = fmaf(a, x.w, acc_wh[k + 3]);
        }
      }
      if (has_emb) {
        const int img0 = __builtin_amdgcn_readfirstlane(img);
        if (__all(img == img0)) {
          float part = 0.f;
#pragma unroll
          for (int s = 0; s < 16; s++) part += rowsH[(wq * 16 + s) * kHP + wi];
          part += __shfl_xor(part, 16);
          part += __shfl_xor(part, 32);
          if (lane < 16) atomicAdd(g_emb + (int64_t)img0 * kOut1 + lane, part);
        } else if (valid) {
#pragma unroll
          for (int i = 0; i < kOut1; i++) atomicAdd(g_emb + (int64_t)img * kOut1 + i, dX[i]);
        }
      }
      wave_lds_sync();
    }
  }

#pragma unroll
  for (int i = 0; i < kIn2; i++) atomicAdd(g_w1 + lane * kIn2 + i, acc_w1[i]);
  atomicAdd(g_b1 + lane, acc_b1);
#pragma unroll
  for (int c = 0; c < 3; c++) atomicAdd(g_w2 + c * kHid + lane, acc_w2[c]);
  {
    const int wi = lane & 15, wq = lane >> 4;
#pragma unroll
    for (int k = 0; k < CQ; k++) atomicAdd(g_w_h + wi * C + wq * CQ + k, acc_wh[k]);
  }
#pragma unroll
  for (int i = 0; i < kOut1; i++) {
    const float t = wave_sum(acc_bh[i]);
    if (lane == 0) atomicAdd(g_b_h + i, t);
  }
#pragma unroll
  for (int c = 0; c < 3; c++) {
    const float t = wave_sum(acc_b2[c]);
    if (lane == 0) atomicAdd(g_b2 + c, t);
  }
}

}

#define F2N_DISPATCH_C(C_, ...)                                   \
  switch (C_) {                                                   \
    case 8: { constexpr int CC = 8; __VA_ARGS__; } break;         \
    case 16: { constexpr int CC = 16; __VA_ARGS__; } break;       \
    case 32: { constexpr int CC = 32; __VA_ARGS__; } break;       \
    case 64: { constexpr int CC = 64; __VA_ARGS__; } break;       \
    default: return F2N_E_UNSUPPORTED;                            \
  }

extern "C" int f2n_shade_fwd(
  const float * enc_cm, int C, const float * dirs, const int32_t * sample_img, const float * w_h,
  const float * b_h, const float * w1, const float * b1, const float * w2, const float * b2,
  const float * app_emb, float * logit, float * rgb, float * pre_cm, int64_t n, void * stream)
{
  if (n < 0) return F2N_E_INVALID_ARG;
  if (C != 8 && C != 16 && C != 32 && C != 64) return F2N_E_UNSUPPORTED;
  if (n == 0) return F2N_OK;
  if (!enc_cm || !dirs || !w_h || !b_h || !w1 || !b1 || !w2 || !b2 || !logit || !rgb)
    return F2N_E_INVALID_ARG;
  if (f2n_get_option(F2N_OPT_SHADE_FWD) == 0 && f2n_detail::shade_bwd_mfma_supports(64, n))
    return f2n_detail::launch_shade_fwd_mfma(
      enc_cm, C, dirs, sample_img, w_h, b_h, w1, b1, w2, b2, app_emb, logit, rgb, pre_cm, n,
      (hipStream_t)stream);
  const dim3 grid(f2n_div_up(n, F2N_BLOCK)), block(F2N_BLOCK);
  F2N_DISPATCH_C(C, hipLaunchKernelGGL(
                      (shade_fwd_kernel<CC>), grid, block, 0, (hipStream_t)stream, enc_cm, dirs,
                      sample_img, w_h, b_h, w1, b1, w2, b2, app_emb, logit, rgb, pre_cm, n))
  return f2n_launch_status();
}

extern "C" int f2n_shade_bwd(
  const float * enc_cm, int C, const float * dirs, const int32_t * sample_img, const float * w_h,
  const float * b_h, const float * w1, const float * b1, const float * w2, const float * b2,
  const float * app_emb, const float * d_logit, const float * d_rgb, float * d_enc_cm,
  float * g_w_h, float * g_b_h, float * g_w1, float * g_b1, float * g_w2, float * g_b2,
  float * g_app_emb, const float * pre_cm, int64_t n, void * stream)
{
  if (n < 0) return F2N_E_INVALID_ARG;
  if (C != 8 && C != 16 && C != 32 && C != 64) return F2N_E_UNSUPPORTED;
  if (n == 0) return F2N_OK;
  if (!enc_cm || !dirs || !w_h || !b_h || !w1 || !b1 || !w2 || !b2 || !d_logit || !d_rgb ||
      !d_enc_cm || !g_w_h || !g_b_h || !g_w1 || !g_b1 || !g_w2 || !g_b2)
    return F2N_E_INVALID_ARG;
  if (app_emb && sample_img && !g_app_emb) return F2N_E_INVALID_ARG;
  const bool force_valu = f2n_get_option(F2N_OPT_SHADE_BWD) == 1;
  if (!force_valu && !pre_cm && f2n_detail::shade_bwd_mfma_supports(C, n))
    return f2n_detail::launch_shade_bwd_mfma(
      enc_cm, C, dirs, sample_img, w_h, b_h, w1, b1, w2, b2, app_emb, d_logit, d_rgb, d_enc_cm,
      g_w_h, g_b_h, g_w1, g_b1, g_w2, g_b2, g_app_emb, n, (hipStream_t)stream);
  const int64_t n_strides = (n + 63) / 64;
  F2N_DISPATCH_C(C, constexpr int kW = BwdShape<CC>::kWaves;
                    const unsigned grid = (unsigned)std::min<int64_t>(256, (n_strides + kW - 1) / kW);
                    hipLaunchKernelGGL(
                      (shade_bwd_kernel<CC>), dim3(grid), dim3(kW * 64), 0,
                      (hipStream_t)stream, enc_cm, dirs, sample_img, w_h, b_h, w1, b1, w2, b2,
                      app_emb, d_logit, d_rgb, d_enc_cm,
                      g_w_h, g_b_h, g_w1, g_b1, g_w2, g_b2, g_app_emb, pre_cm, n))
  return f2n_launch_status();
}
```

### f2-nerf_amd/csrc/kernels/shade_mfma.hip

```cpp
#include "shade_mfma.hiph"

#include "sh_basis.hiph"

#include <cstdlib>

namespace
{

typedef float f32x4 __attribute__((ext_vector_type(4)));

__device__ __forceinline__ f32x4 mfma16(float a, float b, f32x4 c)
{
  return __builtin_amdgcn_mfma_f32_16x16x4f32(a, b, c, 0, 0, 0);
}

constexpr int kOut1 = 16;
constexpr int kIn2 = 32;
constexpr int kHid = 64;
constexpr float kEps = 1e-3f;

template <int C, int TS>
struct MShape
{
  static_assert(C % 8 == 0 && C <= 64, "MFMA path: C must be 8, 16, 32 or 64");
  static_assert(TS == 2 || TS == 4, "16-sample tiles per stride: 2 or 4");
  static constexpr int kStride = 16 * TS;
  static constexpr int kS1 = C / 4;
  static constexpr int kM6 = (C + 15) / 16;
  static constexpr int oWA1 = 0;
  static constexpr int oWA2 = oWA1 + kS1;
  static constexpr int oWA5 = oWA2 + 32;
  static constexpr int oWA6 = oWA5 + 16;
  static constexpr int kSlots = oWA6 + kM6 * 4;
  static constexpr int oW2Q = kSlots * 64;
  static constexpr int oBh = oW2Q + 4 * 4 * 3 * 4;
  static constexpr int oB1 = oBh + 16;
  static constexpr int oB2 = oB1 + 64;
  static constexpr int kWFloats = oB2 + 4;
  static constexpr int kP = (TS == 4) ? 72 : (C == 64) ? 36 : 40;
  static constexpr int oXS = 0;
  static constexpr int oES = oXS + 32 * kP;
  static constexpr int oPS = oES + kM6 * 16 * kP;
  static constexpr int oDS = oPS + 16 * kP;
  static constexpr int kW2M = (TS == 4) ? 4 : 2, kW2R = (TS == 4) ? 4 : 1;
  static constexpr int kAccs = 41 + 3 * kW2M * kW2R + 4 * kM6;
  static constexpr int kWaveFloats =
    (TS == 4 && kAccs * 64 > oDS + 4 * kP) ? kAccs * 64 : oDS + 4 * kP;
  static constexpr int kWaves = (TS == 4) ? 4 : 8;
  static constexpr int kLdsFloats = kWFloats + kWaves * kWaveFloats;
  static_assert(kLdsFloats * 4 <= 160 * 1024, "LDS budget");
  static constexpr int kMeetRegs = kLdsFloats / ((kWaves - 1) * 64);
  static constexpr int kMeetRounds = (kAccs + kMeetRegs - 1) / kMeetRegs;
};

template <int V>
__device__ __forceinline__ void phase_fence_v()
{
  if constexpr (!(V & 1)) __builtin_amdgcn_sched_barrier(0);
}

__device__ __forceinline__ void wave_lds_sync()
{
  __builtin_amdgcn_fence(__ATOMIC_RELEASE, "wavefront");
  __builtin_amdgcn_wave_barrier();
  __builtin_amdgcn_fence(__ATOMIC_ACQUIRE, "wavefront");
}

template <typename T, typename Off>
__device__ __forceinline__ T ld_row(const T * row, Off byte_off)
{
  return *reinterpret_cast<const T *>(reinterpret_cast<const char *>(row) + byte_off);
}
template <typename Off>
__device__ __forceinline__ void st_row(float * row, Off byte_off, float v)
{
  *reinterpret_cast<float *>(reinterpret_cast<char *>(row) + byte_off) = v;
}
template <bool WIDE>
struct RowOffset
{
  typedef uint32_t type;
};
template <>
struct RowOffset<true>
{
  typedef uint64_t type;
};

__device__ __forceinline__ void issue_fence() { __builtin_amdgcn_sched_barrier(0); }

__device__ __forceinline__ float relu(float x)
{
  const int b = __float_as_int(x);
  return __int_as_float(b > 0 ? b : 0);
}

template <int kCtrl>
__device__ __forceinline__ float dpp_move(float v)
{
  return __int_as_float(__builtin_amdgcn_update_dpp(0, __float_as_int(v), kCtrl, 0xf, 0xf, false));
}

__device__ __forceinline__ float quarter_sum(float v)
{
  v += __shfl_xor(v, 8);
  v += __shfl_xor(v, 4);
  v += __shfl_xor(v, 2);
  v += __shfl_xor(v, 1);
  return v;
}

template <int C, int V, bool WIDE, int TS>
__global__ __launch_bounds__((MShape<C, TS>::kWaves * 64)) void shade_bwd_mfma_kernel(
  const float * __restrict__ enc, const float * __restrict__ dirs,
  const int32_t * __restrict__ sample_img, const float * __restrict__ p_w_h,
  const float * __restrict__ p_b_h, const float * __restrict__ p_w1,
  const float * __restrict__ p_b1, const float * __restrict__ p_w2,
  const float * __restrict__ p_b2, const float * __restrict__ p_emb,
  const float * __restrict__ d_logit, const float * __restrict__ d_rgb, float * __restrict__ d_enc,
  float * __restrict__ g_w_h, float * __restrict__ g_b_h, float * __restrict__ g_w1,
  float * __restrict__ g_b1, float * __restrict__ g_w2, float * __restrict__ g_b2,
  float * __restrict__ g_emb, int64_t n)
{
  using S = MShape<C, TS>;
  constexpr int kS1 = S::kS1, kM6 = S::kM6, kP = S::kP, kStride = S::kStride;
  __shared__ __attribute__((aligned(16))) float lds_all[S::kLdsFloats];
  float * lds_w = lds_all;

  for (int i = threadIdx.x; i < S::kSlots * 64; i += S::kWaves * 64) {
    const int slot = i >> 6, l = i & 63, q = l >> 4, m = l & 15;
    float v;
    if (slot < S::oWA2) {
      const int t = slot - S::oWA1;
      v = p_w_h[m * C + q * kS1 + t];
    } else if (slot < S::oWA5) {
      const int M = (slot - S::oWA2) >> 3, t = (slot - S::oWA2) & 7;
      const int k = (t < 4) ? 4 * q + t : 16 + 4 * q + (t - 4);
      v = p_w1[(16 * M + m) * kIn2 + k];
    } else if (slot < S::oWA6) {
      const int M = (slot - S::oWA5) >> 2, r = (slot - S::oWA5) & 3;
      v = p_w1[(16 * M + 4 * q + r) * kIn2 + m];
    } else {
      const int M = (slot - S::oWA6) >> 2, r = (slot - S::oWA6) & 3;
      v = (16 * M + m < C) ? p_w_h[(4 * q + r) * C + 16 * M + m] : 0.f;
    }
    lds_w[i] = v;
  }
  if (threadIdx.x < 192) {
    const int i = threadIdx.x, r = i & 3, c = (i >> 2) % 3, Mq = i / 12;
    lds_w[S::oW2Q + i] = p_w2[c * kHid + 16 * (Mq >> 2) + 4 * (Mq & 3) + r];
  }
  if (threadIdx.x < 16) lds_w[S::oBh + threadIdx.x] = p_b_h[threadIdx.x];
  if (threadIdx.x < 64) lds_w[S::oB1 + threadIdx.x] = p_b1[threadIdx.x];
  if (threadIdx.x < 4) lds_w[S::oB2 + threadIdx.x] = (threadIdx.x < 3) ? p_b2[threadIdx.x] : 0.f;

  const int lane = lane_id();
  const int wave = (int)(threadIdx.x >> 6);
  const int q = lane >> 4, m = lane & 15;
  float * tile = lds_all + S::kWFloats + wave * S::kWaveFloats;
  float * XS = tile + S::oXS;
  float * ES = tile + S::oES;
  float * PS = tile + S::oPS;
  float * DS = tile + S::oDS;
  if constexpr (C % 16 != 0) {
    if (lane < kStride)
      for (int r = C; r < kM6 * 16; r++) ES[r * kP + lane] = 0.f;
  }
  __syncthreads();

  const float * wop = lds_w + lane;
  constexpr bool kWReg = TS == 4 && C <= 32;
  constexpr int kRegLo = S::oWA2, kRegHi = S::oWA5;
  float wreg[kWReg ? kRegHi - kRegLo : 1];
  if constexpr (kWReg) {
#pragma unroll
    for (int i = kRegLo; i < kRegHi; i++) wreg[i - kRegLo] = wop[i * 64];
  }
  auto W = [&](int slot) {
    const bool in_reg = kWReg && slot >= kRegLo && slot < kRegHi;
    return in_reg ? wreg[in_reg ? slot - kRegLo : 0] : wop[slot * 64];
  };
  using Off = typename RowOffset<WIDE>::type;
  const Off cE = (Off)((int64_t)(q * kS1) * n * 4), cD = (Off)((int64_t)(4 * q) * n * 4);
  const bool has_emb = (p_emb != nullptr) && (sample_img != nullptr);

  const f32x4 zero4 = {0.f, 0.f, 0.f, 0.f};
  f32x4 acc_w1[4][2];
  constexpr int kW2M = S::kW2M, kW2R = S::kW2R;
  float acc_w2[3][kW2M][kW2R];
  float w2_even[3];
  f32x4 acc_wh[kM6];
  float acc_b1[4];
  f32x4 acc_bh = zero4;
  float acc_b2 = 0.f;
  f32x4 acc_emb = zero4;
  int emb_img = -1;
  auto flush_emb = [&]() {
    if (emb_img >= 0) {
#pragma unroll
      for (int r = 0; r < 4; r++) {
        const float t = quarter_sum(acc_emb[r]);
        if (m == 0) atomicAdd(g_emb + (int64_t)emb_img * kOut1 + 4 * q + r, t);
      }
    }
    acc_emb = zero4;
  };
#pragma unroll
  for (int M = 0; M < 4; M++) {
    acc_w1[M][0] = acc_w1[M][1] = zero4;
#pragma unroll
    for (int c = 0; c < 3; c++)
#pragma unroll
      for (int r = 0; r < kW2R; r++)
        if (M < kW2M) acc_w2[c][M][r] = 0.f;
    acc_b1[M] = 0.f;
  }
#pragma unroll
  for (int N = 0; N < kM6; N++) acc_wh[N] = zero4;

  const int64_t n_strides = (n + kStride - 1) / kStride;
  const int64_t wave_global = (int64_t)blockIdx.x * S::kWaves + wave;
  const int64_t wave_count = (int64_t)gridDim.x * S::kWaves;
  float eB[kS1][TS];
  int img[TS];
#pragma unroll
  for (int T = 0; T < TS; T++) img[T] = 0;
  float dir[3];
  const int lS = lane % kStride;
  auto load_inputs = [&](int64_t st_, float (&eB_)[kS1][TS], int (&img_)[TS], float (&dir_)[3]) {
    const int64_t s0_ = st_ * kStride;
    uint32_t off_[TS];
#pragma unroll
    for (int T = 0; T < TS; T++) off_[T] = (uint32_t)(((s0_ + 16 * T + m < n) ? s0_ + 16 * T + m : n - 1) * 4);
#pragma unroll
    for (int t = 0; t < kS1; t++)
#pragma unroll
      for (int T = 0; T < TS; T++) eB_[t][T] = ld_row(enc + (int64_t)t * n, off_[T] + cE);
    if (has_emb) {
#pragma unroll
      for (int T = 0; T < TS; T++) img_[T] = ld_row(sample_img, off_[T]);
    }
    const uint32_t offL = (uint32_t)(((s0_ + lS < n) ? s0_ + lS : n - 1) * 12);
#pragma unroll
    for (int k = 0; k < 3; k++) dir_[k] = ld_row(dirs + k, offL);
  };
  if constexpr (TS == 4) {
    load_inputs(wave_global, eB, img, dir);
    issue_fence();
  }

  for (int64_t st = wave_global; st < n_strides; st += wave_count) {
    const int64_t s0 = st * kStride;
    if constexpr (TS == 2) load_inputs(st, eB, img, dir);
    bool vT[TS];
    uint32_t offS[TS];
#pragma unroll
    for (int T = 0; T < TS; T++) {
      const int64_t s = s0 + 16 * T + m;
      vT[T] = s < n;
      offS[T] = (uint32_t)((vT[T] ? s : n - 1) * 4);
    }

    f32x4 h[TS];
#pragma unroll
    for (int T = 0; T < TS; T++) h[T] = *reinterpret_cast<const f32x4 *>(lds_w + S::oBh + 4 * q);
#pragma unroll
    for (int t = 0; t < kS1; t++) {
      const float a = W(S::oWA1 + t);
#pragma unroll
      for (int T = 0; T < TS; T++) h[T] = mfma16(a, eB[t][T], h[T]);
    }
#pragma unroll
    for (int t = 0; t < kS1; t++)
#pragma unroll
      for (int T = 0; T < TS; T++) ES[(q * kS1 + t) * kP + 16 * T + m] = eB[t][T];

    phase_fence_v<V>();
    f32x4 Xh[TS];
    int img_cur[TS];
#pragma unroll
    for (int T = 0; T < TS; T++) img_cur[T] = img[T];
    {
      f32x4 e4[TS];
      if (has_emb) {
#pragma unroll
        for (int T = 0; T < TS; T++)
          e4[T] = *reinterpret_cast<const f32x4 *>(p_emb + (int64_t)img_cur[T] * kOut1 + 4 * q);
      }
      float sh[16];
      sh_basis<4>(dir[0], dir[1], dir[2], sh);
      if constexpr (TS == 4) {
#pragma unroll
        for (int k = 0; k < 16; k++) XS[(16 + k) * kP + lane] = sh[k];
      } else {
        const bool hi = lane >= 32;
#pragma unroll
        for (int k = 0; k < 8; k++) XS[(16 + (hi ? 8 : 0) + k) * kP + lS] = hi ? sh[8 + k] : sh[k];
      }
#pragma unroll
      for (int T = 0; T < TS; T++) {
        Xh[T] = h[T];
        if (q == 0) Xh[T][0] = 1.f;
        if (has_emb) Xh[T] += e4[T];
#pragma unroll
        for (int r = 0; r < 4; r++) XS[(4 * q + r) * kP + 16 * T + m] = Xh[T][r];
      }
    }
    wave_lds_sync();

    phase_fence_v<V>();
    f32x4 pre[4][TS];
    {
      float Xs[4][TS];
#pragma unroll
      for (int t = 0; t < 4; t++)
#pragma unroll
        for (int T = 0; T < TS; T++) Xs[t][T] = XS[(16 + 4 * q + t) * kP + 16 * T + m];
#pragma unroll
      for (int M = 0; M < 4; M++) {
#pragma unroll
        for (int T = 0; T < TS; T++)
          pre[M][T] = *reinterpret_cast<const f32x4 *>(lds_w + S::oB1 + 16 * M + 4 * q);
#pragma unroll
        for (int t = 0; t < 8; t++) {
          const float a = W(S::oWA2 + M * 8 + t);
#pragma unroll
          for (int T = 0; T < TS; T++)
            pre[M][T] = mfma16(a, (t < 4) ? Xh[T][t] : Xs[t - 4][T], pre[M][T]);
        }
      }
    }

    phase_fence_v<V>();
    float d_o[TS];
    {
      float g_rgb[TS];
#pragma unroll
      for (int T = 0; T < TS; T++) g_rgb[T] = ld_row(d_rgb, 3 * offS[T] + ((q < 3) ? 4 * q : 8));
      issue_fence();
      float po[3][TS];
#pragma unroll
      for (int c = 0; c < 3; c++)
#pragma unroll
        for (int T = 0; T < TS; T++) po[c][T] = 0.f;
#pragma unroll
      for (int M = 0; M < 4; M++) {
        f32x4 wq[3];
#pragma unroll
        for (int c = 0; c < 3; c++)
          wq[c] = *reinterpret_cast<const f32x4 *>(lds_w + S::oW2Q + ((M * 4 + q) * 3 + c) * 4);
#pragma unroll
        for (int T = 0; T < TS; T++)
#pragma unroll
          for (int r = 0; r < 4; r++) {
            const float p = relu(pre[M][T][r]);
            pre[M][T][r] = p;
#pragma unroll
            for (int c = 0; c < 3; c++) po[c][T] = __builtin_fmaf(wq[c][r], p, po[c][T]);
          }
      }
      const float b2q = lds_w[S::oB2 + q];
#pragma unroll
      for (int T = 0; T < TS; T++) {
        const float s0 = mfma16(1.f, po[0][T], zero4)[0];
        const float s1 = mfma16(1.f, po[1][T], zero4)[0];
        const float s2 = mfma16(1.f, po[2][T], zero4)[0];
        const float o = ((q == 0) ? s0 : (q == 1) ? s1 : s2) + b2q;
        const float sg = 1.f / (1.f + expf(-o));
        const float g = (vT[T] && q < 3) ? g_rgb[T] : 0.f;
        d_o[T] = g * (1.f + 2.f * kEps) * sg * (1.f - sg);
        acc_b2 += d_o[T];
        if (q < 3) DS[q * kP + 16 * T + m] = d_o[T];
      }
    }
    wave_lds_sync();

    phase_fence_v<V>();
    {
      float doc[3][TS];
#pragma unroll
      for (int c = 0; c < 3; c++)
#pragma unroll
        for (int T = 0; T < TS; T++) doc[c][T] = DS[c * kP + 16 * T + m];
#pragma unroll
      for (int M = 0; M < 4; M++) {
        f32x4 wq[3];
#pragma unroll
        for (int c = 0; c < 3; c++)
          wq[c] = *reinterpret_cast<const f32x4 *>(lds_w + S::oW2Q + ((M * 4 + q) * 3 + c) * 4);
        auto d_hid = [&](int r) {
#pragma unroll
          for (int T = 0; T < TS; T++) {
            float dh = wq[0][r] * doc[0][T];
            dh = __builtin_fmaf(wq[1][r], doc[1][T], dh);
            dh = __builtin_fmaf(wq[2][r], doc[2][T], dh);
            pre[M][T][r] = (pre[M][T][r] > 0.f) ? dh : 0.f;
          }
        };
        if constexpr (kW2R == 4) {
#pragma unroll
          for (int r = 0; r < 4; r++) {
#pragma unroll
            for (int c = 0; c < 3; c++) {
              float t = doc[c][0] * pre[M][0][r];
#pragma unroll
              for (int T = 1; T < TS; T++) t = __builtin_fmaf(doc[c][T], pre[M][T][r], t);
              acc_w2[c][M][r] += t;
            }
            d_hid(r);
          }
        } else {
          float t4[3][4];
#pragma unroll
          for (int r = 0; r < 4; r++)
#pragma unroll
            for (int c = 0; c < 3; c++) {
              float t = doc[c][0] * pre[M][0][r];
#pragma unroll
              for (int T = 1; T < TS; T++) t = __builtin_fmaf(doc[c][T], pre[M][T][r], t);
              t4[c][r] = t;
            }
          const bool lo = m < 8, lo2 = (m & 7) < 4, lo3 = (m & 3) < 2;
#pragma unroll
          for (int c = 0; c < 3; c++) {
            float h2[2];
#pragma unroll
            for (int r = 0; r < 2; r++) {
              const float own = lo ? t4[c][r] : t4[c][r + 2];
              const float give = lo ? t4[c][r + 2] : t4[c][r];
              h2[r] = own + dpp_move<0x140>(give);
            }
            const float own = lo2 ? h2[0] : h2[1];
            const float give = lo2 ? h2[1] : h2[0];
            const float h1 = own + dpp_move<0x141>(give);
            if (M % 2 == 0) {
              w2_even[c] = h1;
            } else {
              const float own3 = lo3 ? w2_even[c] : h1;
              const float give3 = lo3 ? h1 : w2_even[c];
              acc_w2[c][M / 2][0] += own3 + dpp_move<0x4e>(give3);
            }
          }
#pragma unroll
          for (int r = 0; r < 4; r++) d_hid(r);
        }
      }
    }

    phase_fence_v<V>();
    {
      auto put = [&](int M) {
#pragma unroll
        for (int T = 0; T < TS; T++)
#pragma unroll
          for (int r = 0; r < 4; r++) PS[(4 * q + r) * kP + 16 * T + m] = pre[M][T][r];
      };
      put(0);
      wave_lds_sync();
#pragma unroll
      for (int M = 0; M < 4; M++) {
        f32x4 a4[TS];
#pragma unroll
        for (int u = 0; u < TS; u++)
          a4[u] = *reinterpret_cast<const f32x4 *>(PS + m * kP + 16 * u + 4 * q);
        wave_lds_sync();
        if (M < 3) {
          put(M + 1);
          wave_lds_sync();
        }
#pragma unroll
        for (int u = 0; u < TS; u++) {
          acc_b1[M] += (a4[u][0] + a4[u][1]) + (a4[u][2] + a4[u][3]);
          f32x4 b4[2];
#pragma unroll
          for (int N = 0; N < 2; N++)
            b4[N] = *reinterpret_cast<const f32x4 *>(XS + (16 * N + m) * kP + 16 * u + 4 * q);
#pragma unroll
          for (int k = 0; k < 4; k++)
#pragma unroll
            for (int N = 0; N < 2; N++) acc_w1[M][N] = mfma16(a4[u][k], b4[N][k], acc_w1[M][N]);
        }
      }
    }

    if constexpr (TS == 4) {
      load_inputs(st + wave_count, eB, img, dir);
      issue_fence();
    }

    phase_fence_v<V>();
    float g_logit[TS];
#pragma unroll
    for (int T = 0; T < TS; T++) g_logit[T] = ld_row(d_logit, offS[T]);
    issue_fence();
    f32x4 dX[TS];
#pragma unroll
    for (int T = 0; T < TS; T++) dX[T] = zero4;
#pragma unroll
    for (int M = 0; M < 4; M++)
#pragma unroll
      for (int r = 0; r < 4; r++) {
        const float a = W(S::oWA5 + M * 4 + r);
#pragma unroll
        for (int T = 0; T < TS; T++) dX[T] = mfma16(a, pre[M][T][r], dX[T]);
      }

    phase_fence_v<V>();
    if (has_emb) {
      const int img0 = __builtin_amdgcn_readfirstlane(img_cur[0]);
      bool one_img = true;
#pragma unroll
      for (int T = 0; T < TS; T++) one_img = one_img && img_cur[T] == img0;
      if (__all(one_img)) {
        if (img0 != emb_img) {
          flush_emb();
          emb_img = img0;
        }
        if constexpr (TS == 4) acc_emb += (dX[0] + dX[1]) + (dX[2] + dX[3]);
        else acc_emb += dX[0] + dX[1];
      } else {
#pragma unroll
        for (int T = 0; T < TS; T++)
#pragma unroll
          for (int r = 0; r < 4; r++)
            if (vT[T]) atomicAdd(g_emb + (int64_t)img_cur[T] * kOut1 + 4 * q + r, dX[T][r]);
      }
    }

    f32x4 d_h[TS];
#pragma unroll
    for (int T = 0; T < TS; T++) {
      d_h[T] = dX[T];
      if (q == 0) d_h[T][0] = vT[T] ? g_logit[T] : 0.f;
      acc_bh += d_h[T];
#pragma unroll
      for (int r = 0; r < 4; r++) PS[(4 * q + r) * kP + 16 * T + m] = d_h[T][r];
    }

    phase_fence_v<V>();
#pragma unroll
    for (int M = 0; M < kM6; M++) {
      f32x4 de[TS];
#pragma unroll
      for (int T = 0; T < TS; T++) de[T] = zero4;
#pragma unroll
      for (int r = 0; r < 4; r++) {
        const float a = W(S::oWA6 + M * 4 + r);
#pragma unroll
        for (int T = 0; T < TS; T++) de[T] = mfma16(a, d_h[T][r], de[T]);
      }
#pragma unroll
      for (int T = 0; T < TS; T++)
        if (vT[T]) {
#pragma unroll
          for (int r = 0; r < 4; r++)
            if (C % 16 == 0 || 16 * M + 4 * q + r < C)
              st_row(d_enc + (int64_t)(16 * M + r) * n, offS[T] + cD, de[T][r]);
        }
    }

    phase_fence_v<V>();
    wave_lds_sync();
#pragma unroll
    for (int u = 0; u < TS; u++) {
      const f32x4 a4 = *reinterpret_cast<const f32x4 *>(PS + m * kP + 16 * u + 4 * q);
#pragma unroll
      for (int N = 0; N < kM6; N++) {
        const f32x4 b4 = *reinterpret_cast<const f32x4 *>(ES + (16 * N + m) * kP + 16 * u + 4 * q);
#pragma unroll
        for (int k = 0; k < 4; k++) acc_wh[N] = mfma16(a4[k], b4[k], acc_wh[N]);
      }
    }
    wave_lds_sync();
  }

  if (has_emb) flush_emb();
  {
    auto each_acc = [&](auto && fn) {
      int i = 0;
#pragma unroll
      for (int M = 0; M < 4; M++) {
#pragma unroll
        for (int N = 0; N < 2; N++)
#pragma unroll
          for (int r = 0; r < 4; r++) acc_w1[M][N][r] = fn(acc_w1[M][N][r], i++);
        acc_b1[M] = fn(acc_b1[M], i++);
      }
#pragma unroll
      for (int c = 0; c < 3; c++)
#pragma unroll
        for (int M = 0; M < kW2M; M++)
#pragma unroll
          for (int r = 0; r < kW2R; r++) acc_w2[c][M][r] = fn(acc_w2[c][M][r], i++);
#pragma unroll
      for (int N = 0; N < kM6; N++)
#pragma unroll
        for (int r = 0; r < 4; r++) acc_wh[N][r] = fn(acc_wh[N][r], i++);
#pragma unroll
      for (int r = 0; r < 4; r++) acc_bh[r] = fn(acc_bh[r], i++);
      acc_b2 = fn(acc_b2, i++);
    };
    if constexpr (TS == 4) {
      static_assert(S::kAccs * 64 <= S::kWaveFloats, "the accumulators fit a wave's tile region");
      wave_lds_sync();
      if (wave != 0) each_acc([&](float v, int i) { tile[i * 64 + lane] = v; return v; });
      __syncthreads();
      if (wave == 0) {
#pragma unroll
        for (int w = 1; w < S::kWaves; w++) {
          const float * other = lds_all + S::kWFloats + w * S::kWaveFloats;
          each_acc([&](float v, int i) { return v + other[i * 64 + lane]; });
        }
      }
    } else {
      constexpr int R = S::kMeetRegs;
#pragma unroll
      for (int rd = 0; rd < S::kMeetRounds; rd++) {
        const int lo = rd * R, hi = lo + R;
        __syncthreads();
        if (wave != 0)
          each_acc([&](float v, int i) {
            if (i >= lo && i < hi) lds_all[((wave - 1) * R + i - lo) * 64 + lane] = v;
            return v;
          });
        __syncthreads();
        if (wave == 0) {
#pragma unroll
          for (int w = 1; w < S::kWaves; w++)
            each_acc([&](float v, int i) {
              return (i >= lo && i < hi) ? v + lds_all[((w - 1) * R + i - lo) * 64 + lane] : v;
            });
        }
      }
    }
    if (wave != 0) return;
  }
#pragma unroll
  for (int M = 0; M < 4; M++) {
#pragma unroll
    for (int N = 0; N < 2; N++)
#pragma unroll
      for (int r = 0; r < 4; r++)
        atomicAdd(g_w1 + (16 * M + 4 * q + r) * kIn2 + 16 * N + m, acc_w1[M][N][r]);
#pragma unroll
    for (int c = 0; c < 3; c++) {
      if constexpr (kW2R == 4) {
#pragma unroll
        for (int r = 0; r < 4; r++) {
          const float t = quarter_sum(acc_w2[c][M][r]);
          if (m == 0) atomicAdd(g_w2 + c * kHid + 16 * M + 4 * q + r, t);
        }
      } else if (M % 2 == 0) {
        float t = acc_w2[c][M / 2][0];
        t += __shfl_xor(t, 1);
        if ((m & 1) == 0) atomicAdd(g_w2 + c * kHid + 16 * (M + ((m >> 1) & 1)) + 4 * q + (m >> 2), t);
      }
    }
    {
      float t = acc_b1[M];
      t += __shfl_xor(t, 16);
      t += __shfl_xor(t, 32);
      if (q == 0) atomicAdd(g_b1 + 16 * M + m, t);
    }
  }
#pragma unroll
  for (int N = 0; N < kM6; N++)
#pragma unroll
    for (int r = 0; r < 4; r++)
      if (C % 16 == 0 || 16 * N + m < C) atomicAdd(g_w_h + (4 * q + r) * C + 16 * N + m, acc_wh[N][r]);
#pragma unroll
  for (int r = 0; r < 4; r++) {
    const float t = quarter_sum(acc_bh[r]);
    if (m == 0) atomicAdd(g_b_h + 4 * q + r, t);
  }
  {
    const float t = quarter_sum(acc_b2);
    if (m == 0 && q < 3) atomicAdd(g_b2 + q, t);
  }
}


template <int C, int W = 12>
struct FShape
{
  static_assert(C % 8 == 0 && C <= 64, "MFMA path: C must be 8, 16, 32 or 64");
  static constexpr int kS1 = C / 4;
  static constexpr int oWA1 = 0, oWA2 = oWA1 + kS1, oWA3 = oWA2 + 32, kSlots = oWA3 + 16;
  static constexpr int oBh = kSlots * 64, oB1 = oBh + 16, oB2 = oB1 + 64, kWFloats = oB2 + 4;
  static constexpr int kP = 68;
  static constexpr int kWaveFloats = 16 * kP;
  static constexpr int kWaves = W;
  static constexpr int kLdsFloats = kWFloats + kWaves * kWaveFloats;
};

template <int C, bool WIDE, int W>
__global__ __launch_bounds__(W * 64) void shade_fwd_mfma_kernel(
  const float * __restrict__ enc, const float * __restrict__ dirs,
  const int32_t * __restrict__ sample_img, const float * __restrict__ p_w_h,
  const float * __restrict__ p_b_h, const float * __restrict__ p_w1,
  const float * __restrict__ p_b1, const float * __restrict__ p_w2,
  const float * __restrict__ p_b2, const float * __restrict__ p_emb, float * __restrict__ logit,
  float * __restrict__ rgb, float * __restrict__ pre_out, int64_t n)
{
  using S = FShape<C, W>;
  constexpr int kS1 = S::kS1, kP = S::kP;
  __shared__ __attribute__((aligned(16))) float lds_all[S::kLdsFloats];
  float * lds_w = lds_all;
  for (int i = threadIdx.x; i < S::kSlots * 64; i += S::kWaves * 64) {
    const int slot = i >> 6, l = i & 63, q = l >> 4, m = l & 15;
    float v;
    if (slot < S::oWA2) {
      v = p_w_h[m * C + q * kS1 + (slot - S::oWA1)];
    } else if (slot < S::oWA3) {
      const int M = (slot - S::oWA2) >> 3, t = (slot - S::oWA2) & 7;
      v = p_w1[(16 * M + m) * kIn2 + ((t < 4) ? 4 * q + t : 16 + 4 * q + (t - 4))];
    } else {
      const int M = (slot - S::oWA3) >> 2, r = (slot - S::oWA3) & 3;
      v = ((m & 3) == 0 && m < 12) ? p_w2[(m >> 2) * kHid + 16 * M + 4 * q + r] : 0.f;
    }
    lds_w[i] = v;
  }
  if (threadIdx.x < 16) lds_w[S::oBh + threadIdx.x] = p_b_h[threadIdx.x];
  if (threadIdx.x < 64) lds_w[S::oB1 + threadIdx.x] = p_b1[threadIdx.x];
  if (threadIdx.x < 4) lds_w[S::oB2 + threadIdx.x] = (threadIdx.x < 3) ? p_b2[threadIdx.x] : 0.f;
  __syncthreads();

  const int lane = lane_id();
  const int wave = (int)(threadIdx.x >> 6);
  const int q = lane >> 4, m = lane & 15;
  float * XS = lds_all + S::kWFloats + wave * S::kWaveFloats;
  const float * wop = lds_w + lane;
  using Off = typename RowOffset<WIDE>::type;
  const Off cE = (Off)((int64_t)(q * kS1) * n * 4), cP = (Off)((int64_t)(4 * q) * n * 4);
  const bool has_emb = (p_emb != nullptr) && (sample_img != nullptr);
  const f32x4 zero4 = {0.f, 0.f, 0.f, 0.f};

  const int64_t n_strides = (n + 63) / 64;
  const int64_t wave_count = (int64_t)gridDim.x * S::kWaves;
  for (int64_t st = (int64_t)blockIdx.x * S::kWaves + wave; st < n_strides; st += wave_count) {
    const int64_t s0 = st * 64;
    bool vT[4];
    uint32_t offS[4];
#pragma unroll
    for (int T = 0; T < 4; T++) {
      const int64_t s = s0 + 16 * T + m;
      vT[T] = s < n;
      offS[T] = (uint32_t)((vT[T] ? s : n - 1) * 4);
    }
    float eB[kS1][4];
#pragma unroll
    for (int t = 0; t < kS1; t++)
#pragma unroll
      for (int T = 0; T < 4; T++) eB[t][T] = ld_row(enc + (int64_t)t * n, offS[T] + cE);
    int img[4] = {0, 0, 0, 0};
    if (has_emb) {
#pragma unroll
      for (int T = 0; T < 4; T++) img[T] = ld_row(sample_img, offS[T]);
    }
    float dir[3];
    {
      const uint32_t offL = (uint32_t)(((s0 + lane < n) ? s0 + lane : n - 1) * 12);
#pragma unroll
      for (int k = 0; k < 3; k++) dir[k] = ld_row(dirs + k, offL);
    }
    issue_fence();

    f32x4 h[4];
#pragma unroll
    for (int T = 0; T < 4; T++) h[T] = *reinterpret_cast<const f32x4 *>(lds_w + S::oBh + 4 * q);
#pragma unroll
    for (int t = 0; t < kS1; t++) {
      const float a = wop[(S::oWA1 + t) * 64];
#pragma unroll
      for (int T = 0; T < 4; T++) h[T] = mfma16(a, eB[t][T], h[T]);
    }
    if (q == 0) {
#pragma unroll
      for (int T = 0; T < 4; T++)
        if (vT[T]) st_row(logit, offS[T], h[T][0]);
    }

    f32x4 Xh[4];
    {
      f32x4 e4[4];
      if (has_emb) {
#pragma unroll
        for (int T = 0; T < 4; T++)
          e4[T] = *reinterpret_cast<const f32x4 *>(p_emb + (int64_t)img[T] * kOut1 + 4 * q);
      }
      float sh[16];
      sh_basis<4>(dir[0], dir[1], dir[2], sh);
#pragma unroll
      for (int k = 0; k < 16; k++) XS[k * kP + lane] = sh[k];
#pragma unroll
      for (int T = 0; T < 4; T++) {
        Xh[T] = h[T];
        if (q == 0) Xh[T][0] = 1.f;
        if (has_emb) Xh[T] += e4[T];
      }
    }
    wave_lds_sync();
    float Xs[4][4];
#pragma unroll
    for (int t = 0; t < 4; t++)
#pragma unroll
      for (int T = 0; T < 4; T++) Xs[t][T] = XS[(4 * q + t) * kP + 16 * T + m];
    wave_lds_sync();

    f32x4 o[4];
#pragma unroll
    for (int T = 0; T < 4; T++) {
      o[T] = zero4;
      o[T][0] = lds_w[S::oB2 + q];
    }
#pragma unroll
    for (int M = 0; M < 4; M++) {
      f32x4 pre[4];
#pragma unroll
      for (int T = 0; T < 4; T++)
        pre[T] = *reinterpret_cast<const f32x4 *>(lds_w + S::oB1 + 16 * M + 4 * q);
#pragma unroll
      for (int t = 0; t < 8; t++) {
        const float a = wop[(S::oWA2 + M * 8 + t) * 64];
#pragma unroll
        for (int T = 0; T < 4; T++)
          pre[T] = mfma16(a, (t < 4) ? Xh[T][t] : Xs[t - 4][T], pre[T]);
      }
      if (pre_out) {
#pragma unroll
        for (int T = 0; T < 4; T++)
          if (vT[T]) {
#pragma unroll
            for (int r = 0; r < 4; r++)
              st_row(pre_out + (int64_t)(16 * M + r) * n, offS[T] + cP, pre[T][r]);
          }
      }
#pragma unroll
      for (int r = 0; r < 4; r++) {
        const float a = wop[(S::oWA3 + M * 4 + r) * 64];
#pragma unroll
        for (int T = 0; T < 4; T++) o[T] = mfma16(a, relu(pre[T][r]), o[T]);
      }
    }
    if (q < 3) {
#pragma unroll
      for (int T = 0; T < 4; T++)
        if (vT[T])
          st_row(rgb + q, 3 * offS[T], (1.f + 2.f * kEps) / (1.f + expf(-o[T][0])) - kEps);
    }
  }
}

}

namespace f2n_detail
{

constexpr int64_t kShadeBwdTwoWavesMinSamples = F2N_SHADE_BWD_TWO_WAVES_MIN_SAMPLES;

bool shade_bwd_mfma_supports(int C, int64_t n)
{
  return (C == 8 || C == 16 || C == 32 || C == 64) && n < ((int64_t)1 << 28);
}

int launch_shade_bwd_mfma(
  const float * enc_cm, int C, const float * dirs, const int32_t * sample_img, const float * w_h,
  const float * b_h, const float * w1, const float * b1, const float * w2, const float * b2,
  const float * app_emb, const float * d_logit, const float * d_rgb, float * d_enc_cm,
  float * g_w_h, float * g_b_h, float * g_w1, float * g_b1, float * g_w2, float * g_b2,
  float * g_app_emb, int64_t n, hipStream_t stream)
{
  if (app_emb && (reinterpret_cast<uintptr_t>(app_emb) & 15u)) return F2N_E_INVALID_ARG;
  if (n >= ((int64_t)1 << 28)) return F2N_E_UNSUPPORTED;
  const bool wide = (int64_t)C * n >= ((int64_t)1 << 30);
  const int waves = f2n_get_option(F2N_OPT_SHADE_BWD_WAVES);
  const int ts = (waves == 1 || (waves == 0 && n < kShadeBwdTwoWavesMinSamples)) ? 4 : 2;
  const bool mixed = (ts == 4) ? f2n_get_option(F2N_OPT_SHADE_VARIANT) != 1 : waves == 3;
#define F2N_LAUNCH_MFMA_V(CC, VV, WW, TT)                                                            \
  {                                                                                                  \
    using MS = MShape<CC, TT>;                                                                       \
    const int64_t n_strides = (n + MS::kStride - 1) / MS::kStride;                                   \
    const unsigned grid = (unsigned)std::min<int64_t>(256, (n_strides + MS::kWaves - 1) / MS::kWaves); \
    hipLaunchKernelGGL(                                                                              \
      (shade_bwd_mfma_kernel<CC, VV, WW, TT>), dim3(grid), dim3(MS::kWaves * 64), 0, stream, enc_cm, \
      dirs, sample_img, w_h, b_h, w1, b1, w2, b2, app_emb, d_logit, d_rgb, d_enc_cm, g_w_h, g_b_h,   \
      g_w1, g_b1, g_w2, g_b2, g_app_emb, n);                                                         \
  }
#define F2N_LAUNCH_MFMA_T(CC, TT)                            \
  if (wide) F2N_LAUNCH_MFMA_V(CC, (TT == 2 ? 0 : 1), true, TT) \
  else if (mixed) F2N_LAUNCH_MFMA_V(CC, 1, false, TT)        \
  else F2N_LAUNCH_MFMA_V(CC, 0, false, TT)
#define F2N_LAUNCH_MFMA(CC)                                \
  if (ts == 2) { F2N_LAUNCH_MFMA_T(CC, 2) }                \
  else { F2N_LAUNCH_MFMA_T(CC, 4) }
  switch (C) {
    case 8: F2N_LAUNCH_MFMA(8) break;
    case 16: F2N_LAUNCH_MFMA(16) break;
    case 32: F2N_LAUNCH_MFMA(32) break;
    case 64: F2N_LAUNCH_MFMA(64) break;
    default: return F2N_E_UNSUPPORTED;
  }
#undef F2N_LAUNCH_MFMA
#undef F2N_LAUNCH_MFMA_T
#undef F2N_LAUNCH_MFMA_V
  return f2n_launch_status();
}


int launch_shade_fwd_mfma(
  const float * enc_cm, int C, const float * dirs, const int32_t * sample_img, const float * w_h,
  const float * b_h, const float * w1, const float * b1, const float * w2, const float * b2,
  const float * app_emb, float * logit, float * rgb, float * pre_cm, int64_t n, hipStream_t stream)
{
  const int64_t n_strides = (n + 63) / 64;
  if (app_emb && (reinterpret_cast<uintptr_t>(app_emb) & 15u)) return F2N_E_INVALID_ARG;
  if (n >= ((int64_t)1 << 28)) return F2N_E_UNSUPPORTED;
  const bool wide = (int64_t)(pre_cm ? 64 : C) * n >= ((int64_t)1 << 30);
  const bool two_per_simd = f2n_get_option(F2N_OPT_SHADE_VARIANT) == 2;
#define F2N_LAUNCH_FWD_W(CC, WW, KW)                                                               \
  {                                                                                                \
    constexpr int kW = KW;                                                                         \
    const unsigned grid = (unsigned)std::min<int64_t>(256, (n_strides + kW - 1) / kW);             \
    hipLaunchKernelGGL(                                                                            \
      (shade_fwd_mfma_kernel<CC, WW, KW>), dim3(grid), dim3(kW * 64), 0, stream, enc_cm, dirs,     \
      sample_img, w_h, b_h, w1, b1, w2, b2, app_emb, logit, rgb, pre_cm, n);                       \
  }
#define F2N_LAUNCH_FWD(CC)                                                   \
  if (wide) F2N_LAUNCH_FWD_W(CC, true, 12)                                   \
  else if (two_per_simd) F2N_LAUNCH_FWD_W(CC, false, 8)                      \
  else if (f2n_get_option(F2N_OPT_SHADE_VARIANT) == 3) F2N_LAUNCH_FWD_W(CC, false, 12) \
  else F2N_LAUNCH_FWD_W(CC, false, 16)
  switch (C) {
    case 8: F2N_LAUNCH_FWD(8) break;
    case 16: F2N_LAUNCH_FWD(16) break;
    case 32: F2N_LAUNCH_FWD(32) break;
    case 64: F2N_LAUNCH_FWD(64) break;
    default: return F2N_E_UNSUPPORTED;
  }
#undef F2N_LAUNCH_FWD
#undef F2N_LAUNCH_FWD_W
  return f2n_launch_status();
}

}
```

### f2-nerf_amd/csrc/kernels/status.hip

```cpp
#include "common.hiph"

#include <atomic>

namespace
{
std::atomic<int> g_options[F2N_OPT_COUNT];

bool option_value_ok(int key, int value)
{
  switch (key) {
    case F2N_OPT_SHADE_FWD:
    case F2N_OPT_SHADE_BWD:
    case F2N_OPT_BWD_COMBINE:
    case F2N_OPT_BWD_PHASES:
    case F2N_OPT_RAY_ORDER: return value == 0 || value == 1;
    case F2N_OPT_MARCH: return value >= 0 && value <= 2;
    case F2N_OPT_SHADE_BWD_WAVES: return value >= 0 && value <= 3;
    case F2N_OPT_SHADE_VARIANT: return value >= 0 && value <= 3;
    case F2N_OPT_RAYTILE: return value == 0 || value == 16 || value == 32;
    case F2N_OPT_HASH_BWD: return value >= 0 && value <= 2;
    case F2N_OPT_RAYTILE_WALK: return value >= 0 && value <= 3;
    default: return false;
  }
}
}

extern "C" int f2n_set_option(int key, int value)
{
  if (key < 0 || key >= F2N_OPT_COUNT || !option_value_ok(key, value)) return F2N_E_INVALID_ARG;
  return g_options[key].exchange(value, std::memory_order_relaxed);
}

extern "C" int f2n_get_option(int key)
{
  if (key < 0 || key >= F2N_OPT_COUNT) return F2N_E_INVALID_ARG;
  return g_options[key].load(std::memory_order_relaxed);
}

extern "C" int f2n_abi_version(void) { return F2N_ABI_VERSION; }

extern "C" const char * f2n_status_string(int status)
{
  switch (status) {
    case F2N_OK: return "ok";
    case F2N_E_INVALID_ARG: return "invalid argument";
    case F2N_E_LAUNCH: return "kernel launch failed";
    case F2N_E_UNSUPPORTED: return "unsupported configuration";
    default: return "unknown status";
  }
}
```

### include/f2nerf_hip.h

```cpp
#ifndef F2NERF_HIP_H_
#define F2NERF_HIP_H_

#include <stdint.h>

#ifdef __cplusplus
extern "C" {
#endif

#define F2N_ABI_VERSION 2

#define F2N_OK 0
#define F2N_E_INVALID_ARG (-1)
#define F2N_E_LAUNCH (-2)
#define F2N_E_UNSUPPORTED (-3)

#define F2N_MAX_LEVELS 32

int f2n_abi_version(void);
const char * f2n_status_string(int status);

#define F2N_OPT_SHADE_FWD 0
#define F2N_OPT_SHADE_BWD 1
#define F2N_OPT_SHADE_VARIANT 2
#define F2N_OPT_RAYTILE 3
#define F2N_OPT_HASH_BWD 4
#define F2N_OPT_BWD_COMBINE 5
#define F2N_OPT_RAYTILE_WALK 6
#define F2N_OPT_MARCH 7
#define F2N_OPT_BWD_PHASES 8
#define F2N_OPT_RAY_ORDER 9
#define F2N_OPT_SHADE_BWD_WAVES 10
#define F2N_SHADE_BWD_TWO_WAVES_MIN_SAMPLES (3 << 19)
#define F2N_OPT_COUNT 11
int f2n_set_option(int key, int value);
int f2n_get_option(int key);


int f2n_table_to_f16(const float * table_f32, uint16_t * table_f16, int64_t n, void * stream);

int f2n_hash_fwd(
  const float * pts, const uint16_t * table_f16, const int32_t * primes, const float * bias,
  const float * mul, float * out, int64_t out_ld_point, int64_t out_ld_chan, uint32_t * idx_out,
  int64_t n, int L, int F, uint32_t T, int64_t level_stride, void * stream);

int f2n_hash_fwd_raytile(
  const float * pts, const uint16_t * table_f16, const int32_t * primes, const float * bias,
  const float * mul, float * out_cm, int n_rays, int S, int L, int F, uint32_t T,
  int64_t level_stride, void * stream);

int f2n_hash_bwd(
  const float * pts, const uint16_t * table_f16, const int32_t * primes, const float * bias,
  const float * mul, const float * grad_out, int64_t g_ld_point, int64_t g_ld_chan,
  float * table_grad, float * pts_grad, int64_t n, int L, int F, uint32_t T, int64_t level_stride,
  float grad_scale, void * stream);

int64_t f2n_hash_bwd_workspace_bytes(int64_t n, int L, int F, uint32_t T);
int f2n_hash_bwd_set_overflow_counter(uint64_t * device_counter);
int f2n_hash_bwd_binned(
  const float * pts, const int32_t * primes, const float * bias, const float * mul,
  const float * grad_out, int64_t g_ld_point, int64_t g_ld_chan, float * table_grad, int64_t n,
  int L, int F, uint32_t T, int64_t level_stride, float grad_scale, void * workspace,
  int64_t workspace_bytes, void * stream);

int f2n_contract_fwd(const float * pts, float * x, int64_t n, void * stream);
int f2n_contract_bwd(const float * pts, const float * dx, float * dpts, int64_t n, void * stream);

int f2n_hash_rays_grad(
  const float * pts, const float * t, const int32_t * bounds, const float * rays_d,
  const uint16_t * table_f16, const int32_t * primes, const float * bias, const float * mul,
  const float * grad_out, int64_t g_ld_point, int64_t g_ld_chan, float * d_rays_o,
  float * d_rays_d, int n_rays, int L, int F, uint32_t T, int64_t level_stride, float grad_scale,
  void * stream);


int f2n_sh_encode(const float * dirs, float * out, int64_t n, int degree, void * stream);


int f2n_seg_sum_fwd(const float * val, const int32_t * idx, float * sum, int n_rays, void * stream);
int f2n_seg_sum_bwd(const float * dsum, const int32_t * idx, float * dval, int n_rays, void * stream);
int f2n_seg_sum_vec_fwd(
  const float * val, const int32_t * idx, float * sum, int n_rays, int vec, void * stream);
int f2n_seg_sum_vec_bwd(
  const float * dsum, const int32_t * idx, float * dval, int n_rays, int vec, void * stream);
int f2n_seg_scan_fwd(
  const float * val, const int32_t * idx, float * sum, int n_rays, int include_this, void * stream);
int f2n_seg_scan_bwd(
  const float * dsum, const int32_t * idx, float * dval, int n_rays, int include_this,
  void * stream);

int f2n_weight_var_fwd(
  const float * weights, const int32_t * idx, float * out_vars, int n_rays, void * stream);
int f2n_weight_var_bwd(
  const float * weights, const int32_t * idx, const float * dvars, float * dw, int n_rays,
  void * stream);


int f2n_scatter_idx(
  const int32_t * idx, const int32_t * emb_idx, int32_t * all_emb_idx, int n_rays, void * stream);
int f2n_scatter_add_fwd(
  const float * emb, const int32_t * scatter_idx, const float * to_add, float * sum, int64_t n_all,
  int C, void * stream);
int f2n_scatter_add_bwd(
  const int32_t * scatter_idx, const float * dsum, float * demb, int64_t n_all, int n_emb, int C,
  void * stream);


int f2n_gen_rays(
  const float * poses, int pose_ld, const float * intrinsics, int64_t n_cams,
  const int32_t * cam_idx, const int32_t * ij, int64_t first_pixel, int width, float * rays_o,
  float * rays_d, int64_t n, void * stream);

int64_t f2n_gen_rays_bwd_workspace_floats(int64_t n);
int f2n_gen_rays_bwd(
  const float * intrinsics, int64_t n_cams, const int32_t * ij, int64_t first_pixel, int width,
  const float * d_rays_o, const float * d_rays_d, float * d_poses, int pose_ld, float * workspace,
  int64_t n, void * stream);

int f2n_sample_rays(
  const float * rays_o, const float * rays_d, const float * noise, float * pts, float * dirs,
  float * dt, float * t, int32_t * bounds, int n_rays, int S, float step, void * stream);

int f2n_density_march(
  const float * rays_o, const float * rays_d, const float * noise, const uint16_t * table_f16,
  const int32_t * primes, const float * bias, const float * mul, const float * w0, const float * b0,
  int32_t * kept, int n_rays, int S, float step, int L, int F, uint32_t T, int64_t level_stride,
  float t_thresh, float density_shift, void * stream);

int f2n_density_scan(
  const float * enc_cm, int C, const float * dt, const float * w0, const float * b0, int32_t * kept,
  int n_rays, int S, float t_thresh, float density_shift, void * stream);

int f2n_density_margin(
  const float * logit, const float * dt, int32_t * flag, int n_rays, int S, float density_shift,
  float depth_limit, void * stream);

int f2n_compact_rows_cm(
  const float * src, int64_t n_src, float * dst, int64_t n_dst, int C, const int32_t * bounds,
  int n_rays, int S, void * stream);

int f2n_bounds_from_counts(
  const int32_t * kept, int32_t * bounds, int32_t * total, int n_rays, void * stream);

int f2n_sample_compact(
  const float * rays_o, const float * rays_d, const float * noise, const int32_t * bounds,
  float * pts, float * dirs, float * dt, float * t, int n_rays, int S, float step, void * stream);



int f2n_occ_update(
  const uint16_t * table_f16, const int32_t * primes, const float * bias, const float * mul,
  const float * w0, const float * b0, const float * probe_u, float * density, uint32_t * bits, int G,
  int L, int F, uint32_t T, int64_t level_stride, float density_shift, float threshold, float decay,
  void * stream);

int f2n_occ_lookup(
  const float * pts, int64_t n, const uint32_t * bits, int G, uint8_t * out, void * stream);

int f2n_density_march_occ(
  const float * rays_o, const float * rays_d, const float * noise, const uint16_t * table_f16,
  const int32_t * primes, const float * bias, const float * mul, const float * w0, const float * b0,
  const uint32_t * bits, int G, int32_t * kept, int32_t * len, int n_rays, int S, float step, int L,
  int F, uint32_t T, int64_t level_stride, float t_thresh, float density_shift, void * stream);

int f2n_sample_compact_occ(
  const float * rays_o, const float * rays_d, const float * noise, const int32_t * bounds,
  const int32_t * len, const uint32_t * bits, int G, float * pts, float * dirs, float * dt,
  float * t, int n_rays, int S, float step, void * stream);


int f2n_ray_keys(const float * rays_d, int32_t * keys, int n, void * stream);

int f2n_ray_permute(
  const int64_t * order, int n, int S, const float * rays_o, const float * rays_d,
  const int32_t * emb_idx, const float * bg, const float * noise, int32_t * perm, float * rays_o_p,
  float * rays_d_p, int32_t * emb_idx_p, float * bg_p, float * noise_p, int32_t * inv,
  void * stream);

int f2n_gather_rows(
  const float * src, float * dst, const int32_t * map, int n, int row_floats, void * stream);

int f2n_gather_segments(
  const float * src, const int32_t * src_bounds, float * dst, const int32_t * dst_bounds,
  const int32_t * map, int n_rays, void * stream);

int f2n_counts_through(
  const int32_t * bounds, const int32_t * map, int32_t * counts, int n_rays, void * stream);


int f2n_composite_fwd(
  const float * logit, int64_t logit_ld, const float * rgb, const float * dt, const float * t,
  const int32_t * bounds, const float * bg, float * colors, float * depths, float * weights,
  float * last_trans, int n_rays, float density_shift, float t_shift, void * stream);

int f2n_composite_bwd(
  const float * logit, int64_t logit_ld, const float * rgb, const float * dt, const float * t,
  const int32_t * bounds, const float * bg, const float * weights, const float * last_trans,
  const float * d_colors, const float * d_depths, const float * d_weights, float * d_logit,
  float * d_rgb, int n_rays, float density_shift, float t_shift, void * stream);


int f2n_shade_fwd(
  const float * enc_cm, int C, const float * dirs, const int32_t * sample_img, const float * w_h,
  const float * b_h, const float * w1, const float * b1, const float * w2, const float * b2,
  const float * app_emb, float * logit, float * rgb, float * pre_cm, int64_t n, void * stream);

int f2n_shade_bwd(
  const float * enc_cm, int C, const float * dirs, const int32_t * sample_img, const float * w_h,
  const float * b_h, const float * w1, const float * b1, const float * w2, const float * b2,
  const float * app_emb, const float * d_logit, const float * d_rgb, float * d_enc_cm,
  float * g_w_h, float * g_b_h, float * g_w1, float * g_b1, float * g_w2, float * g_b2,
  float * g_app_emb, const float * pre_cm, int64_t n, void * stream);


int f2n_adam_step(
  float * param, const float * grad, float * exp_avg, float * exp_avg_sq, uint16_t * shadow_f16,
  int64_t n, float lr, float beta1, float beta2, float eps, float weight_decay, int step,
  void * stream);

int64_t f2n_loss_workspace_floats(int n_rays);
int f2n_loss_fwd(
  const float * colors, const float * gt, const float * var, int n_rays, float var_weight,
  float * d_colors, float * d_var, float * partial, float * out4, void * stream);


int f2n_perturb_poses(
  const float * pose, int pose_ld, const float * noise, float sigma_pos_x, float sigma_pos_y,
  float sigma_pos_z, float sigma_rot_x, float sigma_rot_y, float sigma_rot_z, float * poses, int P,
  void * stream);

int f2n_pose_scores(
  const float * colors, const float * image, const int32_t * ij, float * loss, float * weights,
  double * workspace, int P, int K, int h, int w, void * stream);

int f2n_average_pose(
  const float * poses, const float * weights, float * pose_out, int P, void * stream);

#ifdef __cplusplus
}
#endif

#endif
```

Measured before the change: 11.57 million rays/s.

## Add ray-uniform shade path exploiting per-ray constant direction and embedding

Adds a ray-aware shading forward/backward path used when every ray has exactly S samples, with S a multiple of 64. Direction, spherical-harmonic basis and appearance embedding are then constant across each 64-sample stride. The kernels load the direction and image id once per stride and fold the SH part of the first layer into a shared bias computed once. They also reduce bias gradients per stride and skip the per-sample ScatterIdx kernel and some LDS syncs. This adds a templated RAYS variant and more kernel instantiations, and it depends on samples staying ray-contiguous and dense.

```diff
diff --git a/f2-nerf_amd/csrc/host/ragged_ops.cpp b/f2-nerf_amd/csrc/host/ragged_ops.cpp
--- a/f2-nerf_amd/csrc/host/ragged_ops.cpp
+++ b/f2-nerf_amd/csrc/host/ragged_ops.cpp
@@ -327,6 +327,101 @@
   }
 };
 
+class ShadeRaysFn : public torch::autograd::Function<ShadeRaysFn>
+{
+public:
+  static variable_list forward(
+    AutogradContext * ctx, Tensor enc, Tensor dirs, Tensor ray_img, int64_t S, Tensor w_h,
+    Tensor b_h, Tensor w1, Tensor b1, Tensor w2, Tensor b2, Tensor app_emb)
+  {
+    TORCH_CHECK(enc.is_cuda() && enc.scalar_type() == torch::kFloat32 && enc.dim() == 2, "enc");
+    const int64_t n = enc.size(0);
+    const int C = (int)enc.size(1);
+    TORCH_CHECK(S > 0 && S % 64 == 0 && n % S == 0 && n < ((int64_t)1 << 28), "shade_rays: n = n_rays * S, S % 64 == 0");
+    const int n_rays = (int)(n / S);
+    Tensor enc_cm = as_channel_major(enc);
+    dirs = f2n::dev_f32(dirs.detach(), "shade dirs");
+    TORCH_CHECK(dirs.numel() == n * 3, "shade_rays: dirs [n, 3]");
+    const bool use_emb =
+      ray_img.defined() && app_emb.defined() && ray_img.numel() > 0 && app_emb.numel() > 0;
+    if (use_emb) {
+      ray_img = f2n::dev_i32(ray_img, "shade ray_img");
+      TORCH_CHECK(ray_img.numel() == n_rays, "shade_rays: ray_img [n_rays]");
+    }
+    w_h = f2n::dev_f32(w_h, "w_h");
+    b_h = f2n::dev_f32(b_h, "b_h");
+    w1 = f2n::dev_f32(w1, "w1");
+    b1 = f2n::dev_f32(b1, "b1");
+    w2 = f2n::dev_f32(w2, "w2");
+    b2 = f2n::dev_f32(b2, "b2");
+    Tensor emb = use_emb ? f2n::dev_f32(app_emb, "app_emb") : Tensor();
+    TORCH_CHECK(
+      w_h.size(0) == 16 && w_h.size(1) == C && w1.size(0) == 64 && w1.size(1) == 32 &&
+        w2.size(0) == 3 && w2.size(1) == 64,
+      "shade: layer shapes must be 16xC, 64x32, 3x64");
+    Tensor logit = torch::empty({n}, enc.options()), rgb = torch::empty({n, 3}, enc.options());
+    {
+    f2n::ScopedKernelTimer timer("shade_fwd", f2n::current_stream(enc_cm), (double)n);
+    f2n::check(
+      f2n_shade_fwd_rays(
+        enc_cm.data_ptr<float>(), C, dirs.data_ptr<float>(), use_emb ? f2n::iptr(ray_img) : nullptr,
+        f2n::fptr(w_h), f2n::fptr(b_h), f2n::fptr(w1), f2n::fptr(b1), f2n::fptr(w2), f2n::fptr(b2),
+        f2n::fptr(emb), logit.data_ptr<float>(), rgb.data_ptr<float>(), n_rays, (int)S,
+        f2n::current_stream(enc_cm)),
+      "f2n_shade_fwd_rays");
+    }
+    ctx->save_for_backward(
+      {enc_cm, dirs, use_emb ? ray_img : Tensor(), w_h, b_h, w1, b1, w2, b2, emb});
+    ctx->saved_data["S"] = S;
+    return {logit, rgb};
+  }
+
+  static variable_list backward(AutogradContext * ctx, variable_list grad_output)
+  {
+    auto sv = ctx->get_saved_variables();
+    Tensor &enc_cm = sv[0], &dirs = sv[1], &ray_img = sv[2], &w_h = sv[3], &b_h = sv[4],
+           &w1 = sv[5], &b1 = sv[6], &w2 = sv[7], &b2 = sv[8], &emb = sv[9];
+    const int C = (int)enc_cm.size(0);
+    const int64_t n = enc_cm.size(1), S = ctx->saved_data["S"].toInt();
+    auto opt = enc_cm.options();
+    Tensor d_logit = grad_output[0].defined() ? f2n::dev_f32(grad_output[0], "d_logit")
+                                              : torch::zeros({n}, opt);
+    Tensor d_rgb = grad_output[1].defined() ? f2n::dev_f32(grad_output[1], "d_rgb")
+                                            : torch::zeros({n, 3}, opt);
+    Tensor d_enc_cm = torch::empty({(int64_t)C, n}, opt);
+    const bool use_emb = emb.defined() && ray_img.defined();
+    auto pad4 = [](int64_t v) { return (v + 3) / 4 * 4; };
+    const int64_t sizes[7] = {w_h.numel(), b_h.numel(), w1.numel(), b1.numel(),
+                              w2.numel(), b2.numel(), use_emb ? emb.numel() : 0};
+    int64_t total = 0;
+    for (int64_t v : sizes) total += pad4(v);
+    Tensor gbuf = torch::zeros({total}, opt);
+    int64_t off = 0;
+    auto take = [&](const Tensor & like, int64_t numel) {
+      Tensor v = gbuf.narrow(0, off, numel).view(like.sizes());
+      off += pad4(numel);
+      return v;
+    };
+    Tensor g_w_h = take(w_h, sizes[0]), g_b_h = take(b_h, sizes[1]), g_w1 = take(w1, sizes[2]),
+           g_b1 = take(b1, sizes[3]), g_w2 = take(w2, sizes[4]), g_b2 = take(b2, sizes[5]);
+    Tensor g_emb = use_emb ? take(emb, sizes[6]) : Tensor();
+    {
+    f2n::ScopedKernelTimer timer("shade_bwd", f2n::current_stream(enc_cm), (double)n);
+    f2n::check(
+      f2n_shade_bwd_rays(
+        enc_cm.data_ptr<float>(), C, dirs.data_ptr<float>(), use_emb ? f2n::iptr(ray_img) : nullptr,
+        f2n::fptr(w_h), f2n::fptr(b_h), f2n::fptr(w1), f2n::fptr(b1), f2n::fptr(w2), f2n::fptr(b2),
+        f2n::fptr(emb), f2n::fptr(d_logit), f2n::fptr(d_rgb), d_enc_cm.data_ptr<float>(),
+        g_w_h.data_ptr<float>(), g_b_h.data_ptr<float>(), g_w1.data_ptr<float>(),
+        g_b1.data_ptr<float>(), g_w2.data_ptr<float>(), g_b2.data_ptr<float>(),
+        use_emb ? g_emb.data_ptr<float>() : nullptr, (int)(n / S), (int)S,
+        f2n::current_stream(enc_cm)),
+      "f2n_shade_bwd_rays");
+    }
+    return {d_enc_cm.t(), Tensor(), Tensor(), Tensor(), g_w_h, g_b_h, g_w1, g_b1, g_w2, g_b2, g_emb};
+  }
+};
+
 
 class TrainLossFn : public torch::autograd::Function<TrainLossFn>
 {
@@ -409,6 +504,7 @@
   idx_start_end = f2n::dev_i32(idx_start_end, "CustomOps::ScatterIdx idx_start_end");
   emb_idx = f2n::dev_i32(emb_idx, "CustomOps::ScatterIdx emb_idx");
   Tensor ret = torch::empty({n_all_pts}, idx_start_end.options());
+  f2n::ScopedKernelTimer timer("scatter_idx", f2n::current_stream(idx_start_end), (double)n_all_pts);
   f2n::check(
     f2n_scatter_idx(
       f2n::iptr(idx_start_end), f2n::iptr(emb_idx), ret.data_ptr<int32_t>(),
@@ -430,6 +526,26 @@
   return {out[0], out[1]};
 }
 
+f2n::ShadeOut f2n::shade_rays(
+  const Tensor & enc, const Tensor & dirs, const Tensor & ray_img, int64_t S, const Tensor & w_h,
+  const Tensor & b_h, const Tensor & w1, const Tensor & b1, const Tensor & w2, const Tensor & b2,
+  const Tensor & app_emb)
+{
+  const Tensor no_img = torch::empty({0}, f2n::int_on(enc.device()));
+  const Tensor no_emb = torch::empty({0, 16}, enc.options());
+  const bool use_emb = ray_img.defined() && app_emb.defined();
+  auto out = ShadeRaysFn::apply(
+    enc, dirs, use_emb ? ray_img : no_img, S, w_h, b_h, w1, b1, w2, b2, use_emb ? app_emb : no_emb);
+  return {out[0], out[1]};
+}
+
+bool f2n::shade_rays_applies(int64_t n, int64_t n_rays, int64_t S)
+{
+  return n_rays > 0 && S > 0 && S % 64 == 0 && n == n_rays * S && n < ((int64_t)1 << 28) &&
+         f2n_get_option(F2N_OPT_SHADE_RAYS) == 0 && f2n_get_option(F2N_OPT_SHADE_FWD) == 0 &&
+         f2n_get_option(F2N_OPT_SHADE_BWD) == 0;
+}
+
 f2n::CompositeOut f2n::composite(
   const Tensor & field_out, const Tensor & rgb, const Tensor & dt, const Tensor & t,
   const Tensor & idx_start_end, const Tensor & bg_color, bool bounds_tile_samples)
diff --git a/f2-nerf_amd/csrc/host/ragged_ops.hpp b/f2-nerf_amd/csrc/host/ragged_ops.hpp
--- a/f2-nerf_amd/csrc/host/ragged_ops.hpp
+++ b/f2-nerf_amd/csrc/host/ragged_ops.hpp
@@ -53,6 +53,13 @@
   const Tensor & b_h, const Tensor & w1, const Tensor & b1, const Tensor & w2, const Tensor & b2,
   const Tensor & app_emb);
 
+ShadeOut shade_rays(
+  const Tensor & enc, const Tensor & dirs, const Tensor & ray_img, int64_t S, const Tensor & w_h,
+  const Tensor & b_h, const Tensor & w1, const Tensor & b1, const Tensor & w2, const Tensor & b2,
+  const Tensor & app_emb);
+
+bool shade_rays_applies(int64_t n, int64_t n_rays, int64_t S);
+
 Tensor train_loss(
   const Tensor & colors, const Tensor & gt_colors, const Tensor & var, float var_loss_weight);
 
diff --git a/f2-nerf_amd/csrc/host/renderer.cpp b/f2-nerf_amd/csrc/host/renderer.cpp
--- a/f2-nerf_amd/csrc/host/renderer.cpp
+++ b/f2-nerf_amd/csrc/host/renderer.cpp
@@ -604,13 +604,21 @@
       enc, route.grad_rays.origins, route.grad_rays.dirs, kept.pts, kept.t, kept.pts_idx_bounds,
       torch::IValue(info))[0];
   }
+  auto mlp = shader_->mlp_params();
+  const Tensor emb = mode == RunningMode::TRAIN ? app_emb_ : Tensor();
+  const int64_t n_rays = kept.pts_idx_bounds.size(0), S = pts_sampler_->options_.max_samples;
+  if (f2n::shade_rays_applies(n_kept, n_rays, S)) {
+    f2n::ShadeOut sh = f2n::shade_rays(
+      enc, kept.dirs, mode == RunningMode::TRAIN ? emb_idx : Tensor(), S,
+      scene_field_->mlp_->weight, scene_field_->mlp_->bias, mlp[0], mlp[1], mlp[2], mlp[3], emb);
+    return {sh.logit.unsqueeze(1), sh.rgb};
+  }
   Tensor sample_img;
   if (mode == RunningMode::TRAIN)
     sample_img = CustomOps::ScatterIdx((int)n_kept, kept.pts_idx_bounds, emb_idx);
-  auto mlp = shader_->mlp_params();
   f2n::ShadeOut sh = f2n::shade(
     enc, kept.dirs, sample_img, scene_field_->mlp_->weight, scene_field_->mlp_->bias, mlp[0],
-    mlp[1], mlp[2], mlp[3], mode == RunningMode::TRAIN ? app_emb_ : Tensor());
+    mlp[1], mlp[2], mlp[3], emb);
   return {sh.logit.unsqueeze(1), sh.rgb};
 }
 
diff --git a/f2-nerf_amd/csrc/kernels/shade.hip b/f2-nerf_amd/csrc/kernels/shade.hip
--- a/f2-nerf_amd/csrc/kernels/shade.hip
+++ b/f2-nerf_amd/csrc/kernels/shade.hip
@@ -468,3 +468,40 @@
                       g_w_h, g_b_h, g_w1, g_b1, g_w2, g_b2, g_app_emb, pre_cm, n))
   return f2n_launch_status();
 }
+
+
+extern "C" int f2n_shade_fwd_rays(
+  const float * enc_cm, int C, const float * dirs, const int32_t * ray_img, const float * w_h,
+  const float * b_h, const float * w1, const float * b1, const float * w2, const float * b2,
+  const float * app_emb, float * logit, float * rgb, int n_rays, int S, void * stream)
+{
+  if (n_rays < 0 || S <= 0 || S % 64 != 0) return F2N_E_INVALID_ARG;
+  if (C != 8 && C != 16 && C != 32 && C != 64) return F2N_E_UNSUPPORTED;
+  if (n_rays == 0) return F2N_OK;
+  if (!enc_cm || !dirs || !w_h || !b_h || !w1 || !b1 || !w2 || !b2 || !logit || !rgb)
+    return F2N_E_INVALID_ARG;
+  if (!f2n_detail::shade_bwd_mfma_supports(C, (int64_t)n_rays * S)) return F2N_E_UNSUPPORTED;
+  return f2n_detail::launch_shade_fwd_mfma_rays(
+    enc_cm, C, dirs, ray_img, w_h, b_h, w1, b1, w2, b2, app_emb, logit, rgb, n_rays, S,
+    (hipStream_t)stream);
+}
+
+extern "C" int f2n_shade_bwd_rays(
+  const float * enc_cm, int C, const float * dirs, const int32_t * ray_img, const float * w_h,
+  const float * b_h, const float * w1, const float * b1, const float * w2, const float * b2,
+  const float * app_emb, const float * d_logit, const float * d_rgb, float * d_enc_cm,
+  float * g_w_h, float * g_b_h, float * g_w1, float * g_b1, float * g_w2, float * g_b2,
+  float * g_app_emb, int n_rays, int S, void * stream)
+{
+  if (n_rays < 0 || S <= 0 || S % 64 != 0) return F2N_E_INVALID_ARG;
+  if (C != 8 && C != 16 && C != 32 && C != 64) return F2N_E_UNSUPPORTED;
+  if (n_rays == 0) return F2N_OK;
+  if (!enc_cm || !dirs || !w_h || !b_h || !w1 || !b1 || !w2 || !b2 || !d_logit || !d_rgb ||
+      !d_enc_cm || !g_w_h || !g_b_h || !g_w1 || !g_b1 || !g_w2 || !g_b2)
+    return F2N_E_INVALID_ARG;
+  if (app_emb && ray_img && !g_app_emb) return F2N_E_INVALID_ARG;
+  if (!f2n_detail::shade_bwd_mfma_supports(C, (int64_t)n_rays * S)) return F2N_E_UNSUPPORTED;
+  return f2n_detail::launch_shade_bwd_mfma_rays(
+    enc_cm, C, dirs, ray_img, w_h, b_h, w1, b1, w2, b2, app_emb, d_logit, d_rgb, d_enc_cm, g_w_h,
+    g_b_h, g_w1, g_b1, g_w2, g_b2, g_app_emb, n_rays, S, (hipStream_t)stream);
+}
diff --git a/f2-nerf_amd/csrc/kernels/shade_mfma.hip b/f2-nerf_amd/csrc/kernels/shade_mfma.hip
--- a/f2-nerf_amd/csrc/kernels/shade_mfma.hip
+++ b/f2-nerf_amd/csrc/kernels/shade_mfma.hip
@@ -101,6 +101,12 @@
   return __int_as_float(__builtin_amdgcn_update_dpp(0, __float_as_int(v), kCtrl, 0xf, 0xf, false));
 }
 
+__device__ __forceinline__ float pick4(int i, float a, float b, float c, float d)
+{
+  const float lo = (i & 1) ? b : a, hi = (i & 1) ? d : c;
+  return (i & 2) ? hi : lo;
+}
+
 __device__ __forceinline__ float quarter_sum(float v)
 {
   v += __shfl_xor(v, 8);
@@ -110,8 +116,8 @@
   return v;
 }
 
-template <int C, int V, bool WIDE, int TS>
-__global__ __launch_bounds__((MShape<C, TS>::kWaves * 64)) void shade_bwd_mfma_kernel(
+template <int C, int V, bool WIDE, int TS, bool RAYS>
+__device__ __forceinline__ void shade_bwd_mfma_body(
   const float * __restrict__ enc, const float * __restrict__ dirs,
   const int32_t * __restrict__ sample_img, const float * __restrict__ p_w_h,
   const float * __restrict__ p_b_h, const float * __restrict__ p_w1,
@@ -120,7 +126,7 @@
   const float * __restrict__ d_logit, const float * __restrict__ d_rgb, float * __restrict__ d_enc,
   float * __restrict__ g_w_h, float * __restrict__ g_b_h, float * __restrict__ g_w1,
   float * __restrict__ g_b1, float * __restrict__ g_w2, float * __restrict__ g_b2,
-  float * __restrict__ g_emb, int64_t n)
+  float * __restrict__ g_emb, int64_t n, int n_per_ray)
 {
   using S = MShape<C, TS>;
   constexpr int kS1 = S::kS1, kM6 = S::kM6, kP = S::kP, kStride = S::kStride;
@@ -155,7 +161,7 @@
   if (threadIdx.x < 4) lds_w[S::oB2 + threadIdx.x] = (threadIdx.x < 3) ? p_b2[threadIdx.x] : 0.f;
 
   const int lane = lane_id();
-  const int wave = (int)(threadIdx.x >> 6);
+  const int wave = RAYS ? __builtin_amdgcn_readfirstlane((int)(threadIdx.x >> 6)) : (int)(threadIdx.x >> 6);
   const int q = lane >> 4, m = lane & 15;
   float * tile = lds_all + S::kWFloats + wave * S::kWaveFloats;
   float * XS = tile + S::oXS;
@@ -229,6 +235,21 @@
   const int lS = lane % kStride;
   auto load_inputs = [&](int64_t st_, float (&eB_)[kS1][TS], int (&img_)[TS], float (&dir_)[3]) {
     const int64_t s0_ = st_ * kStride;
+    if constexpr (RAYS) {
+      const uint32_t sc = (uint32_t)((s0_ < n) ? s0_ : n - kStride);
+#pragma unroll
+      for (int t = 0; t < kS1; t++)
+#pragma unroll
+        for (int T = 0; T < TS; T++) eB_[t][T] = ld_row(enc + (int64_t)t * n, (sc + 16 * T + m) * 4 + cE);
+      if (has_emb) {
+        const int id = sample_img[sc / (uint32_t)n_per_ray];
+#pragma unroll
+        for (int T = 0; T < TS; T++) img_[T] = id;
+      }
+#pragma unroll
+      for (int k = 0; k < 3; k++) dir_[k] = dirs[(int64_t)sc * 3 + k];
+      return;
+    }
     uint32_t off_[TS];
 #pragma unroll
     for (int T = 0; T < TS; T++) off_[T] = (uint32_t)(((s0_ + 16 * T + m < n) ? s0_ + 16 * T + m : n - 1) * 4);
@@ -257,7 +278,7 @@
 #pragma unroll
     for (int T = 0; T < TS; T++) {
       const int64_t s = s0 + 16 * T + m;
-      vT[T] = s < n;
+      vT[T] = RAYS || s < n;
       offS[T] = (uint32_t)((vT[T] ? s : n - 1) * 4);
     }
 
@@ -280,16 +301,25 @@
     int img_cur[TS];
 #pragma unroll
     for (int T = 0; T < TS; T++) img_cur[T] = img[T];
+    float shq[4], shm = 0.f;
     {
       f32x4 e4[TS];
       if (has_emb) {
 #pragma unroll
         for (int T = 0; T < TS; T++)
-          e4[T] = *reinterpret_cast<const f32x4 *>(p_emb + (int64_t)img_cur[T] * kOut1 + 4 * q);
+          if (!RAYS || T == 0)
+            e4[T] = *reinterpret_cast<const f32x4 *>(p_emb + (int64_t)img_cur[T] * kOut1 + 4 * q);
       }
       float sh[16];
       sh_basis<4>(dir[0], dir[1], dir[2], sh);
-      if constexpr (TS == 4) {
+      if constexpr (RAYS) {
+#pragma unroll
+        for (int t = 0; t < 4; t++)
+          shq[t] = pick4(q, sh[t], sh[4 + t], sh[8 + t], sh[12 + t]);
+        shm = pick4(
+          m >> 2, pick4(m & 3, sh[0], sh[1], sh[2], sh[3]), pick4(m & 3, sh[4], sh[5], sh[6], sh[7]),
+          pick4(m & 3, sh[8], sh[9], sh[10], sh[11]), pick4(m & 3, sh[12], sh[13], sh[14], sh[15]));
+      } else if constexpr (TS == 4) {
 #pragma unroll
         for (int k = 0; k < 16; k++) XS[(16 + k) * kP + lane] = sh[k];
       } else {
@@ -301,16 +331,35 @@
       for (int T = 0; T < TS; T++) {
         Xh[T] = h[T];
         if (q == 0) Xh[T][0] = 1.f;
-        if (has_emb) Xh[T] += e4[T];
+        if (has_emb) Xh[T] += e4[RAYS ? 0 : T];
 #pragma unroll
         for (int r = 0; r < 4; r++) XS[(4 * q + r) * kP + 16 * T + m] = Xh[T][r];
       }
     }
-    wave_lds_sync();
+    if constexpr (!RAYS) wave_lds_sync();
 
     phase_fence_v<V>();
     f32x4 pre[4][TS];
-    {
+    if constexpr (RAYS) {
+#pragma unroll
+      for (int M = 0; M < 4; M++)
+        pre[M][0] = *reinterpret_cast<const f32x4 *>(lds_w + S::oB1 + 16 * M + 4 * q);
+#pragma unroll
+      for (int t = 4; t < 8; t++)
+#pragma unroll
+        for (int M = 0; M < 4; M++) pre[M][0] = mfma16(W(S::oWA2 + M * 8 + t), shq[t - 4], pre[M][0]);
+#pragma unroll
+      for (int M = 0; M < 4; M++) {
+#pragma unroll
+        for (int T = 1; T < TS; T++) pre[M][T] = pre[M][0];
+#pragma unroll
+        for (int t = 0; t < 4; t++) {
+          const float a = W(S::oWA2 + M * 8 + t);
+#pragma unroll
+          for (int T = 0; T < TS; T++) pre[M][T] = mfma16(a, Xh[T][t], pre[M][T]);
+        }
+      }
+    } else {
       float Xs[4][TS];
 #pragma unroll
       for (int t = 0; t < 4; t++)
@@ -468,17 +517,25 @@
           put(M + 1);
           wave_lds_sync();
         }
+        constexpr int kN = RAYS ? 1 : 2;
+        float db = 0.f;
 #pragma unroll
         for (int u = 0; u < TS; u++) {
-          acc_b1[M] += (a4[u][0] + a4[u][1]) + (a4[u][2] + a4[u][3]);
-          f32x4 b4[2];
-#pragma unroll
-          for (int N = 0; N < 2; N++)
+          const float su = (a4[u][0] + a4[u][1]) + (a4[u][2] + a4[u][3]);
+          if constexpr (RAYS) db += su;
+          else acc_b1[M] += su;
+          f32x4 b4[kN];
+#pragma unroll
+          for (int N = 0; N < kN; N++)
             b4[N] = *reinterpret_cast<const f32x4 *>(XS + (16 * N + m) * kP + 16 * u + 4 * q);
 #pragma unroll
           for (int k = 0; k < 4; k++)
 #pragma unroll
-            for (int N = 0; N < 2; N++) acc_w1[M][N] = mfma16(a4[u][k], b4[N][k], acc_w1[M][N]);
+            for (int N = 0; N < kN; N++) acc_w1[M][N] = mfma16(a4[u][k], b4[N][k], acc_w1[M][N]);
+        }
+        if constexpr (RAYS) {
+          acc_b1[M] += db;
+          acc_w1[M][1] = mfma16(db, shm, acc_w1[M][1]);
         }
       }
     }
@@ -509,9 +566,11 @@
     if (has_emb) {
       const int img0 = __builtin_amdgcn_readfirstlane(img_cur[0]);
       bool one_img = true;
-#pragma unroll
-      for (int T = 0; T < TS; T++) one_img = one_img && img_cur[T] == img0;
-      if (__all(one_img)) {
+      if constexpr (!RAYS) {
+#pragma unroll
+        for (int T = 0; T < TS; T++) one_img = one_img && img_cur[T] == img0;
+      }
+      if (RAYS || __all(one_img)) {
         if (img0 != emb_img) {
           flush_emb();
           emb_img = img0;
@@ -679,6 +738,35 @@
   }
 }
 
+#define F2N_SHADE_BWD_PARAMS(IMG)                                                                     \
+  const float * __restrict__ enc, const float * __restrict__ dirs, const int32_t * __restrict__ IMG,  \
+    const float * __restrict__ p_w_h, const float * __restrict__ p_b_h,                               \
+    const float * __restrict__ p_w1, const float * __restrict__ p_b1,                                 \
+    const float * __restrict__ p_w2, const float * __restrict__ p_b2,                                 \
+    const float * __restrict__ p_emb, const float * __restrict__ d_logit,                             \
+    const float * __restrict__ d_rgb, float * __restrict__ d_enc, float * __restrict__ g_w_h,         \
+    float * __restrict__ g_b_h, float * __restrict__ g_w1, float * __restrict__ g_b1,                 \
+    float * __restrict__ g_w2, float * __restrict__ g_b2, float * __restrict__ g_emb
+#define F2N_SHADE_BWD_ARGS(IMG)                                                                       \
+  enc, dirs, IMG, p_w_h, p_b_h, p_w1, p_b1, p_w2, p_b2, p_emb, d_logit, d_rgb, d_enc, g_w_h, g_b_h,    \
+    g_w1, g_b1, g_w2, g_b2, g_emb
+
+template <int C, int V, bool WIDE, int TS>
+__global__ __launch_bounds__((MShape<C, TS>::kWaves * 64)) void shade_bwd_mfma_kernel(
+  F2N_SHADE_BWD_PARAMS(sample_img), int64_t n)
+{
+  shade_bwd_mfma_body<C, V, WIDE, TS, false>(F2N_SHADE_BWD_ARGS(sample_img), n, 0);
+}
+
+template <int C, int V, bool WIDE, int TS>
+__global__ __launch_bounds__((MShape<C, TS>::kWaves * 64)) void shade_bwd_mfma_rays_kernel(
+  F2N_SHADE_BWD_PARAMS(ray_img), int64_t n, int S)
+{
+  shade_bwd_mfma_body<C, V, WIDE, TS, true>(F2N_SHADE_BWD_ARGS(ray_img), n, S);
+}
+#undef F2N_SHADE_BWD_PARAMS
+#undef F2N_SHADE_BWD_ARGS
+
 
 template <int C, int W = 12>
 struct FShape
@@ -693,18 +781,18 @@
   static constexpr int kLdsFloats = kWFloats + kWaves * kWaveFloats;
 };
 
-template <int C, bool WIDE, int W>
-__global__ __launch_bounds__(W * 64) void shade_fwd_mfma_kernel(
+template <int C, bool WIDE, int W, bool RAYS>
+__device__ __forceinline__ void shade_fwd_mfma_body(
   const float * __restrict__ enc, const float * __restrict__ dirs,
   const int32_t * __restrict__ sample_img, const float * __restrict__ p_w_h,
   const float * __restrict__ p_b_h, const float * __restrict__ p_w1,
   const float * __restrict__ p_b1, const float * __restrict__ p_w2,
   const float * __restrict__ p_b2, const float * __restrict__ p_emb, float * __restrict__ logit,
-  float * __restrict__ rgb, float * __restrict__ pre_out, int64_t n)
+  float * __restrict__ rgb, float * __restrict__ pre_out, int64_t n, int n_per_ray)
 {
   using S = FShape<C, W>;
   constexpr int kS1 = S::kS1, kP = S::kP;
-  __shared__ __attribute__((aligned(16))) float lds_all[S::kLdsFloats];
+  __shared__ __attribute__((aligned(16))) float lds_all[RAYS ? S::kWFloats : S::kLdsFloats];
   float * lds_w = lds_all;
   for (int i = threadIdx.x; i < S::kSlots * 64; i += S::kWaves * 64) {
     const int slot = i >> 6, l = i & 63, q = l >> 4, m = l & 15;
@@ -726,9 +814,9 @@
   __syncthreads();
 
   const int lane = lane_id();
-  const int wave = (int)(threadIdx.x >> 6);
+  const int wave = RAYS ? __builtin_amdgcn_readfirstlane((int)(threadIdx.x >> 6)) : (int)(threadIdx.x >> 6);
   const int q = lane >> 4, m = lane & 15;
-  float * XS = lds_all + S::kWFloats + wave * S::kWaveFloats;
+  float * XS = lds_all + (RAYS ? 0 : S::kWFloats + wave * S::kWaveFloats);
   const float * wop = lds_w + lane;
   using Off = typename RowOffset<WIDE>::type;
   const Off cE = (Off)((int64_t)(q * kS1) * n * 4), cP = (Off)((int64_t)(4 * q) * n * 4);
@@ -744,7 +832,7 @@
 #pragma unroll
     for (int T = 0; T < 4; T++) {
       const int64_t s = s0 + 16 * T + m;
-      vT[T] = s < n;
+      vT[T] = RAYS || s < n;
       offS[T] = (uint32_t)((vT[T] ? s : n - 1) * 4);
     }
     float eB[kS1][4];
@@ -753,12 +841,16 @@
 #pragma unroll
       for (int T = 0; T < 4; T++) eB[t][T] = ld_row(enc + (int64_t)t * n, offS[T] + cE);
     int img[4] = {0, 0, 0, 0};
-    if (has_emb) {
-#pragma unroll
-      for (int T = 0; T < 4; T++) img[T] = ld_row(sample_img, offS[T]);
-    }
     float dir[3];
-    {
+    if constexpr (RAYS) {
+      if (has_emb) img[0] = sample_img[(uint32_t)s0 / (uint32_t)n_per_ray];
+#pragma unroll
+      for (int k = 0; k < 3; k++) dir[k] = dirs[s0 * 3 + k];
+    } else {
+      if (has_emb) {
+#pragma unroll
+        for (int T = 0; T < 4; T++) img[T] = ld_row(sample_img, offS[T]);
+      }
       const uint32_t offL = (uint32_t)(((s0 + lane < n) ? s0 + lane : n - 1) * 12);
 #pragma unroll
       for (int k = 0; k < 3; k++) dir[k] = ld_row(dirs + k, offL);
@@ -781,31 +873,40 @@
     }
 
     f32x4 Xh[4];
+    float Xs[4][4];
     {
       f32x4 e4[4];
       if (has_emb) {
 #pragma unroll
         for (int T = 0; T < 4; T++)
-          e4[T] = *reinterpret_cast<const f32x4 *>(p_emb + (int64_t)img[T] * kOut1 + 4 * q);
+          if (!RAYS || T == 0)
+            e4[T] = *reinterpret_cast<const f32x4 *>(p_emb + (int64_t)img[T] * kOut1 + 4 * q);
       }
       float sh[16];
       sh_basis<4>(dir[0], dir[1], dir[2], sh);
-#pragma unroll
-      for (int k = 0; k < 16; k++) XS[k * kP + lane] = sh[k];
+      if constexpr (RAYS) {
+#pragma unroll
+        for (int t = 0; t < 4; t++)
+          Xs[t][0] = pick4(q, sh[t], sh[4 + t], sh[8 + t], sh[12 + t]);
+      } else {
+#pragma unroll
+        for (int k = 0; k < 16; k++) XS[k * kP + lane] = sh[k];
+      }
 #pragma unroll
       for (int T = 0; T < 4; T++) {
         Xh[T] = h[T];
         if (q == 0) Xh[T][0] = 1.f;
-        if (has_emb) Xh[T] += e4[T];
-      }
-    }
-    wave_lds_sync();
-    float Xs[4][4];
-#pragma unroll
-    for (int t = 0; t < 4; t++)
-#pragma unroll
-      for (int T = 0; T < 4; T++) Xs[t][T] = XS[(4 * q + t) * kP + 16 * T + m];
-    wave_lds_sync();
+        if (has_emb) Xh[T] += e4[RAYS ? 0 : T];
+      }
+    }
+    if constexpr (!RAYS) {
+      wave_lds_sync();
+#pragma unroll
+      for (int t = 0; t < 4; t++)
+#pragma unroll
+        for (int T = 0; T < 4; T++) Xs[t][T] = XS[(4 * q + t) * kP + 16 * T + m];
+      wave_lds_sync();
+    }
 
     f32x4 o[4];
 #pragma unroll
@@ -816,17 +917,31 @@
 #pragma unroll
     for (int M = 0; M < 4; M++) {
       f32x4 pre[4];
-#pragma unroll
-      for (int T = 0; T < 4; T++)
-        pre[T] = *reinterpret_cast<const f32x4 *>(lds_w + S::oB1 + 16 * M + 4 * q);
-#pragma unroll
-      for (int t = 0; t < 8; t++) {
-        const float a = wop[(S::oWA2 + M * 8 + t) * 64];
+      if constexpr (RAYS) {
+        f32x4 c = *reinterpret_cast<const f32x4 *>(lds_w + S::oB1 + 16 * M + 4 * q);
+#pragma unroll
+        for (int t = 4; t < 8; t++) c = mfma16(wop[(S::oWA2 + M * 8 + t) * 64], Xs[t - 4][0], c);
+#pragma unroll
+        for (int T = 0; T < 4; T++) pre[T] = c;
+#pragma unroll
+        for (int t = 0; t < 4; t++) {
+          const float a = wop[(S::oWA2 + M * 8 + t) * 64];
+#pragma unroll
+          for (int T = 0; T < 4; T++) pre[T] = mfma16(a, Xh[T][t], pre[T]);
+        }
+      } else {
 #pragma unroll
         for (int T = 0; T < 4; T++)
-          pre[T] = mfma16(a, (t < 4) ? Xh[T][t] : Xs[t - 4][T], pre[T]);
-      }
-      if (pre_out) {
+          pre[T] = *reinterpret_cast<const f32x4 *>(lds_w + S::oB1 + 16 * M + 4 * q);
+#pragma unroll
+        for (int t = 0; t < 8; t++) {
+          const float a = wop[(S::oWA2 + M * 8 + t) * 64];
+#pragma unroll
+          for (int T = 0; T < 4; T++)
+            pre[T] = mfma16(a, (t < 4) ? Xh[T][t] : Xs[t - 4][T], pre[T]);
+        }
+      }
+      if (!RAYS && pre_out) {
 #pragma unroll
         for (int T = 0; T < 4; T++)
           if (vT[T]) {
@@ -851,6 +966,30 @@
   }
 }
 
+#define F2N_SHADE_FWD_PARAMS(IMG)                                                                     \
+  const float * __restrict__ enc, const float * __restrict__ dirs, const int32_t * __restrict__ IMG,  \
+    const float * __restrict__ p_w_h, const float * __restrict__ p_b_h,                               \
+    const float * __restrict__ p_w1, const float * __restrict__ p_b1,                                 \
+    const float * __restrict__ p_w2, const float * __restrict__ p_b2,                                 \
+    const float * __restrict__ p_emb, float * __restrict__ logit, float * __restrict__ rgb
+
+template <int C, bool WIDE, int W>
+__global__ __launch_bounds__(W * 64) void shade_fwd_mfma_kernel(
+  F2N_SHADE_FWD_PARAMS(sample_img), float * __restrict__ pre_out, int64_t n)
+{
+  shade_fwd_mfma_body<C, WIDE, W, false>(
+    enc, dirs, sample_img, p_w_h, p_b_h, p_w1, p_b1, p_w2, p_b2, p_emb, logit, rgb, pre_out, n, 0);
+}
+
+template <int C, bool WIDE, int W>
+__global__ __launch_bounds__(W * 64) void shade_fwd_mfma_rays_kernel(
+  F2N_SHADE_FWD_PARAMS(ray_img), int64_t n, int S)
+{
+  shade_fwd_mfma_body<C, WIDE, W, true>(
+    enc, dirs, ray_img, p_w_h, p_b_h, p_w1, p_b1, p_w2, p_b2, p_emb, logit, rgb, nullptr, n, S);
+}
+#undef F2N_SHADE_FWD_PARAMS
+
 }
 
 namespace f2n_detail
@@ -863,28 +1002,37 @@
   return (C == 8 || C == 16 || C == 32 || C == 64) && n < ((int64_t)1 << 28);
 }
 
-int launch_shade_bwd_mfma(
-  const float * enc_cm, int C, const float * dirs, const int32_t * sample_img, const float * w_h,
+static int launch_shade_bwd_mfma_any(
+  const float * enc_cm, int C, const float * dirs, const int32_t * img, const float * w_h,
   const float * b_h, const float * w1, const float * b1, const float * w2, const float * b2,
   const float * app_emb, const float * d_logit, const float * d_rgb, float * d_enc_cm,
   float * g_w_h, float * g_b_h, float * g_w1, float * g_b1, float * g_w2, float * g_b2,
-  float * g_app_emb, int64_t n, hipStream_t stream)
+  float * g_app_emb, int64_t n, int S, hipStream_t stream)
 {
   if (app_emb && (reinterpret_cast<uintptr_t>(app_emb) & 15u)) return F2N_E_INVALID_ARG;
   if (n >= ((int64_t)1 << 28)) return F2N_E_UNSUPPORTED;
   const bool wide = (int64_t)C * n >= ((int64_t)1 << 30);
   const int waves = f2n_get_option(F2N_OPT_SHADE_BWD_WAVES);
-  const int ts = (waves == 1 || (waves == 0 && n < kShadeBwdTwoWavesMinSamples)) ? 4 : 2;
+  const bool rays_one_wave = S > 0 && wide && C == 64;
+  const int ts =
+    (waves == 1 || (waves == 0 && n < kShadeBwdTwoWavesMinSamples) || rays_one_wave) ? 4 : 2;
   const bool mixed = (ts == 4) ? f2n_get_option(F2N_OPT_SHADE_VARIANT) != 1 : waves == 3;
 #define F2N_LAUNCH_MFMA_V(CC, VV, WW, TT)                                                            \
   {                                                                                                  \
     using MS = MShape<CC, TT>;                                                                       \
     const int64_t n_strides = (n + MS::kStride - 1) / MS::kStride;                                   \
     const unsigned grid = (unsigned)std::min<int64_t>(256, (n_strides + MS::kWaves - 1) / MS::kWaves); \
-    hipLaunchKernelGGL(                                                                              \
-      (shade_bwd_mfma_kernel<CC, VV, WW, TT>), dim3(grid), dim3(MS::kWaves * 64), 0, stream, enc_cm, \
-      dirs, sample_img, w_h, b_h, w1, b1, w2, b2, app_emb, d_logit, d_rgb, d_enc_cm, g_w_h, g_b_h,   \
-      g_w1, g_b1, g_w2, g_b2, g_app_emb, n);                                                         \
+    if (S > 0) {                                                                                     \
+      if constexpr (!(CC == 64 && WW && TT == 2))                                 \
+        hipLaunchKernelGGL(                                                                          \
+          (shade_bwd_mfma_rays_kernel<CC, VV, WW, TT>), dim3(grid), dim3(MS::kWaves * 64), 0,        \
+          stream, enc_cm, dirs, img, w_h, b_h, w1, b1, w2, b2, app_emb, d_logit, d_rgb, d_enc_cm,    \
+          g_w_h, g_b_h, g_w1, g_b1, g_w2, g_b2, g_app_emb, n, S);                                    \
+    } else                                                                                           \
+      hipLaunchKernelGGL(                                                                            \
+        (shade_bwd_mfma_kernel<CC, VV, WW, TT>), dim3(grid), dim3(MS::kWaves * 64), 0, stream,       \
+        enc_cm, dirs, img, w_h, b_h, w1, b1, w2, b2, app_emb, d_logit, d_rgb, d_enc_cm, g_w_h,       \
+        g_b_h, g_w1, g_b1, g_w2, g_b2, g_app_emb, n);                                                \
   }
 #define F2N_LAUNCH_MFMA_T(CC, TT)                            \
   if (wide) F2N_LAUNCH_MFMA_V(CC, (TT == 2 ? 0 : 1), true, TT) \
@@ -906,11 +1054,37 @@
   return f2n_launch_status();
 }
 
-
-int launch_shade_fwd_mfma(
+int launch_shade_bwd_mfma(
   const float * enc_cm, int C, const float * dirs, const int32_t * sample_img, const float * w_h,
   const float * b_h, const float * w1, const float * b1, const float * w2, const float * b2,
-  const float * app_emb, float * logit, float * rgb, float * pre_cm, int64_t n, hipStream_t stream)
+  const float * app_emb, const float * d_logit, const float * d_rgb, float * d_enc_cm,
+  float * g_w_h, float * g_b_h, float * g_w1, float * g_b1, float * g_w2, float * g_b2,
+  float * g_app_emb, int64_t n, hipStream_t stream)
+{
+  return launch_shade_bwd_mfma_any(
+    enc_cm, C, dirs, sample_img, w_h, b_h, w1, b1, w2, b2, app_emb, d_logit, d_rgb, d_enc_cm, g_w_h,
+    g_b_h, g_w1, g_b1, g_w2, g_b2, g_app_emb, n, 0, stream);
+}
+
+int launch_shade_bwd_mfma_rays(
+  const float * enc_cm, int C, const float * dirs, const int32_t * ray_img, const float * w_h,
+  const float * b_h, const float * w1, const float * b1, const float * w2, const float * b2,
+  const float * app_emb, const float * d_logit, const float * d_rgb, float * d_enc_cm,
+  float * g_w_h, float * g_b_h, float * g_w1, float * g_b1, float * g_w2, float * g_b2,
+  float * g_app_emb, int n_rays, int S, hipStream_t stream)
+{
+  if (S <= 0 || S % 64 != 0 || n_rays <= 0) return F2N_E_INVALID_ARG;
+  return launch_shade_bwd_mfma_any(
+    enc_cm, C, dirs, ray_img, w_h, b_h, w1, b1, w2, b2, app_emb, d_logit, d_rgb, d_enc_cm, g_w_h,
+    g_b_h, g_w1, g_b1, g_w2, g_b2, g_app_emb, (int64_t)n_rays * S, S, stream);
+}
+
+
+static int launch_shade_fwd_mfma_any(
+  const float * enc_cm, int C, const float * dirs, const int32_t * img, const float * w_h,
+  const float * b_h, const float * w1, const float * b1, const float * w2, const float * b2,
+  const float * app_emb, float * logit, float * rgb, float * pre_cm, int64_t n, int S,
+  hipStream_t stream)
 {
   const int64_t n_strides = (n + 63) / 64;
   if (app_emb && (reinterpret_cast<uintptr_t>(app_emb) & 15u)) return F2N_E_INVALID_ARG;
@@ -921,9 +1095,14 @@
   {                                                                                                \
     constexpr int kW = KW;                                                                         \
     const unsigned grid = (unsigned)std::min<int64_t>(256, (n_strides + kW - 1) / kW);             \
-    hipLaunchKernelGGL(                                                                            \
-      (shade_fwd_mfma_kernel<CC, WW, KW>), dim3(grid), dim3(kW * 64), 0, stream, enc_cm, dirs,     \
-      sample_img, w_h, b_h, w1, b1, w2, b2, app_emb, logit, rgb, pre_cm, n);                       \
+    if (S > 0)                                                                                     \
+      hipLaunchKernelGGL(                                                                          \
+        (shade_fwd_mfma_rays_kernel<CC, WW, KW>), dim3(grid), dim3(kW * 64), 0, stream, enc_cm,    \
+        dirs, img, w_h, b_h, w1, b1, w2, b2, app_emb, logit, rgb, n, S);                           \
+    else                                                                                           \
+      hipLaunchKernelGGL(                                                                          \
+        (shade_fwd_mfma_kernel<CC, WW, KW>), dim3(grid), dim3(kW * 64), 0, stream, enc_cm, dirs,   \
+        img, w_h, b_h, w1, b1, w2, b2, app_emb, logit, rgb, pre_cm, n);                            \
   }
 #define F2N_LAUNCH_FWD(CC)                                                   \
   if (wide) F2N_LAUNCH_FWD_W(CC, true, 12)                                   \
@@ -942,4 +1121,24 @@
   return f2n_launch_status();
 }
 
-}
+int launch_shade_fwd_mfma(
+  const float * enc_cm, int C, const float * dirs, const int32_t * sample_img, const float * w_h,
+  const float * b_h, const float * w1, const float * b1, const float * w2, const float * b2,
+  const float * app_emb, float * logit, float * rgb, float * pre_cm, int64_t n, hipStream_t stream)
+{
+  return launch_shade_fwd_mfma_any(
+    enc_cm, C, dirs, sample_img, w_h, b_h, w1, b1, w2, b2, app_emb, logit, rgb, pre_cm, n, 0, stream);
+}
+
+int launch_shade_fwd_mfma_rays(
+  const float * enc_cm, int C, const float * dirs, const int32_t * ray_img, const float * w_h,
+  const float * b_h, const float * w1, const float * b1, const float * w2, const float * b2,
+  const float * app_emb, float * logit, float * rgb, int n_rays, int S, hipStream_t stream)
+{
+  if (S <= 0 || S % 64 != 0 || n_rays <= 0) return F2N_E_INVALID_ARG;
+  return launch_shade_fwd_mfma_any(
+    enc_cm, C, dirs, ray_img, w_h, b_h, w1, b1, w2, b2, app_emb, logit, rgb, nullptr,
+    (int64_t)n_rays * S, S, stream);
+}
+
+}
diff --git a/f2-nerf_amd/csrc/kernels/status.hip b/f2-nerf_amd/csrc/kernels/status.hip
--- a/f2-nerf_amd/csrc/kernels/status.hip
+++ b/f2-nerf_amd/csrc/kernels/status.hip
@@ -13,7 +13,8 @@
     case F2N_OPT_SHADE_BWD:
     case F2N_OPT_BWD_COMBINE:
     case F2N_OPT_BWD_PHASES:
-    case F2N_OPT_RAY_ORDER: return value == 0 || value == 1;
+    case F2N_OPT_RAY_ORDER:
+    case F2N_OPT_SHADE_RAYS: return value == 0 || value == 1;
     case F2N_OPT_MARCH: return value >= 0 && value <= 2;
     case F2N_OPT_SHADE_BWD_WAVES: return value >= 0 && value <= 3;
     case F2N_OPT_SHADE_VARIANT: return value >= 0 && value <= 3;
diff --git a/include/f2nerf_hip.h b/include/f2nerf_hip.h
--- a/include/f2nerf_hip.h
+++ b/include/f2nerf_hip.h
@@ -31,7 +31,8 @@
 #define F2N_OPT_RAY_ORDER 9
 #define F2N_OPT_SHADE_BWD_WAVES 10
 #define F2N_SHADE_BWD_TWO_WAVES_MIN_SAMPLES (3 << 19)
-#define F2N_OPT_COUNT 11
+#define F2N_OPT_SHADE_RAYS 11
+#define F2N_OPT_COUNT 12
 int f2n_set_option(int key, int value);
 int f2n_get_option(int key);
 
@@ -211,6 +212,18 @@
   float * g_w_h, float * g_b_h, float * g_w1, float * g_b1, float * g_w2, float * g_b2,
   float * g_app_emb, const float * pre_cm, int64_t n, void * stream);
 
+int f2n_shade_fwd_rays(
+  const float * enc_cm, int C, const float * dirs, const int32_t * ray_img, const float * w_h,
+  const float * b_h, const float * w1, const float * b1, const float * w2, const float * b2,
+  const float * app_emb, float * logit, float * rgb, int n_rays, int S, void * stream);
+
+int f2n_shade_bwd_rays(
+  const float * enc_cm, int C, const float * dirs, const int32_t * ray_img, const float * w_h,
+  const float * b_h, const float * w1, const float * b1, const float * w2, const float * b2,
+  const float * app_emb, const float * d_logit, const float * d_rgb, float * d_enc_cm,
+  float * g_w_h, float * g_b_h, float * g_w1, float * g_b1, float * g_w2, float * g_b2,
+  float * g_app_emb, int n_rays, int S, void * stream);
+
 
 int f2n_adam_step(
   float * param, const float * grad, float * exp_avg, float * exp_avg_sq, uint16_t * shadow_f16,
```

Measured after the change: 12.35 million rays/s, median of 6. 6.8% higher.
